# loehnea/bensolve

Hardware: AMD Instinct MI355X
Metric: scalar LPs/sec (Benson phase 2, batched P2(v) solves incl. cut application), synthetic VLP q=5 n=500 m=1000 (higher is better)
Workload: dtype f64

## Files before the change

### bensolve_amd/csrc/poly_engine.hip

```cpp
#include "common.h"
#include <vector>
#include <chrono>
#include <algorithm>
#include <cmath>
#include <thread>
#include <atomic>
#include <cstddef>

namespace bslv {

constexpr int MAXD = 16;
constexpr double POLY_EPS = 1e-9;
constexpr int PB = 256;
constexpr unsigned char F_USED = 1, F_IDEAL = 2, F_SLTN = 4;
constexpr int CRING = 1024;
constexpr int CSTRIDE = 8;
constexpr int LCAP = 16;
constexpr int LONGN = 64;
constexpr int ZMAX = 8;

struct Hp { double h[MAXD + 1]; };
struct Tri { int a, b, c; };

struct PolyView {
// ... 1387 lines not shown
                    if (it * WAVE >= nn) break;
                    const unsigned long long bm = __ballot(k[it]);
                    if (k[it]) {
                        P.pool[on + base + __popcll(bm & ((1ull << lane) - 1ull))] = g[it];
                        if (!row) P.keep[oo + it * WAVE + lane] = 0;
                        if (lb) atomicOr(&lb[g[it] >> 5], 1u << (g[it] & 31));
                    }
                    base += __popcll(bm);
                }
            } else
            for (int j0 = 0; j0 < nn; j0 += WAVE) {
                const int j = j0 + lane;
                const int g = j < nn ? P.pool[oo + j] : 0;
                const bool k = j < nn && (row ? row[g] == Z.stamp : P.keep[oo + j] != 0);
                const unsigned long long bm = __ballot(k);
                if (k) {
                    P.pool[on + base + __popcll(bm & ((1ull << lane) - 1ull))] = g;
                    if (!row) P.keep[oo + j] = 0;
                    if (lb) atomicOr(&lb[g >> 5], 1u << (g & 31));
                }
                base += __popcll(bm);
            }
            if (lane == 0) {
                P.pool[on + base] = facet; P.inc_off[vv] = on; P.inc_len[vv] = base + 1; if (lb) atomicOr(&lb[facet >> 5], 1u << (facet & 31));
                if (rm > 0) P.capx[vv] = ((unsigned long long)on << 32) | (unsigned)rm;
            }
        }
    }
    if (!valid) return;
    if (c == -1) { P.flag[i] &= ~F_USED; return; }
    if (c != 0) return;
    members[ex.a] = i;
    if (longz) return;
    int m = 0;
    if (n <= LCAP) {
        int lst[LCAP];
        unsigned keptmask = 0;
        const unsigned char *K = P.keep + off_old;
        load_list(P.pool + off_old, n, lst);
#pragma unroll
        for (int j = 0; j < LCAP; j++) { unsigned k = (j < n) ? K[j] : 0; keptmask |= (k & 1u) << j; }
#pragma unroll
        for (int j = 0; j < LCAP; j++) if ((keptmask >> j) & 1u) { P.pool[off_new + m++] = lst[j]; P.keep[off_old + j] = 0; }
    } else
        for (int j = 0; j < n; j++)
            if (P.keep[off_old + j]) { P.pool[off_new + m++] = P.pool[off_old + j]; P.keep[off_old + j] = 0; }
    P.pool[off_new + m++] = facet;
    P.inc_off[i] = off_new;
    P.inc_len[i] = m;
    relist_bitmap(P, i, off_new, m);
}

constexpr int K2T = 1024, K2_MAXNM = 512, K2_MAXLONG = 64;
constexpr int K2_HASH_LOG = 13, K2_HASH = 1 << K2_HASH_LOG;
__device__ __forceinline__ void pair_decode32(int p, int nm, int &i, int &j)
{
    const float b2 = 2.0f * nm - 1.0f;
    int ii = (int)((b2 - sqrtf(b2 * b2 - 8.0f * (float)p)) * 0.5f);
    ii = ii < 0 ? 0 : (ii > nm - 2 ? nm - 2 : ii);
    while (ii * (2 * nm - ii - 1) / 2 > p) ii--;
    while ((ii + 1) * (2 * nm - ii - 2) / 2 <= p) ii++;
    i = ii;
    j = ii + 1 + (p - ii * (2 * nm - ii - 1) / 2);
}
template <class F>
__device__ __forceinline__ void k2_for_entries(const int *pool, int nm, const unsigned *s_off, const int *s_len, const unsigned char *s_islong,
                                               const int *s_long, int nlong, F f)
{
    for (int m = threadIdx.x / LPM; m < nm; m += K2T / LPM) {
        if (s_islong[m]) continue;
        const int *L = pool + s_off[m];
        const int n = s_len[m];
        for (int j = threadIdx.x % LPM; j < n; j += LPM) f(m, L[j]);
    }
    for (int k = 0; k < nlong; k++) {
        const int m = s_long[k];
        const int *L = pool + s_off[m];
        const int n = s_len[m];
        for (int j = threadIdx.x; j < n; j += K2T) f(m, L[j]);
    }
}
template <int NWC>
__device__ __forceinline__ void k2_pairs(int nm, int d, int W, int NW, const unsigned long long *bits, const unsigned long long *rows, unsigned *adj_bits,
                                         int (*queue)[128], const unsigned long long *later = nullptr)
{
    const int lane = threadIdx.x & 63, wave = threadIdx.x >> 6;
    auto sweep = [&](int p) {
        int i, j;
        pair_decode32(p, nm, i, j);
        unsigned long long acc[NWC];
#pragma unroll
        for (int k = 0; k < NWC; k++) acc[k] = ~0ull;
        for (int w = 0; w < W; w++) {
            unsigned long long M = bits[w * nm + i] & bits[w * nm + j];
            while (M) {
                const int f = (w << 6) + __ffsll((long long)M) - 1;
                M &= M - 1;
#pragma unroll
                for (int k = 0; k < NWC; k++) acc[k] &= (NWC == 1 || k < NW) ? rows[f * NW + k] : 0ull;
            }
        }
        int cnt = 0;
#pragma unroll
        for (int k = 0; k < NWC; k++) cnt += __popcll(acc[k]);
        if (cnt == 2) atomicOr(&adj_bits[p >> 5], 1u << (p & 31));
    };
    int qn = 0;
    int *q = queue[wave];
    for (int i = wave; i < nm - 1; i += K2T / WAVE) {
        const int rowbase = i * (2 * nm - i - 1) / 2 - (i + 1);
        for (int j0 = i + 1; j0 < nm; j0 += WAVE) {
            const int j = j0 + lane;
            bool cand = false;
            if (j < nm) {
                int nmut = 0;
                unsigned long long lat = 0ull;
                for (int w = 0; w < W; w++) { const unsigned long long x = bits[w * nm + i] & bits[w * nm + j]; nmut += __popcll(x); if (later) lat |= x & later[w]; }
                if (d == 1) atomicOr(&adj_bits[(rowbase + j) >> 5], 1u << ((rowbase + j) & 31));
                else cand = nmut >= d - 1 && lat == 0ull;
            }
            const unsigned long long bm = __ballot(cand);
            if (bm == 0ull) continue;
            if (cand) q[qn + __popcll(bm & ((1ull << lane) - 1ull))] = rowbase + j;
            qn += __popcll(bm);
            __builtin_amdgcn_fence(__ATOMIC_SEQ_CST, "wavefront");
            if (qn >= WAVE) {
                qn -= WAVE;
                sweep(q[qn + lane]);
                __builtin_amdgcn_fence(__ATOMIC_SEQ_CST, "wavefront");
            }
        }
    }
    if (lane < qn) sweep(q[lane]);
}
struct RState;
struct K2V2 {
    const RState *st; const int *cutof; int *mem_g; unsigned *adj_g; int *cnt_g; int *nm_g; int adjw_cap; long long *pair_tests;
    int *fc2, *fl2, *fc_ticket; int fc_slices, fc_stride;
};
__device__ __forceinline__ int k2v2_round(const RState *st);
__device__ __forceinline__ int k2v2_rank_base(const RState *st);
__device__ __forceinline__ bool k2v2_member(const PolyView &P, int v, int co, int vs, int want)
{
    if (co >= -1) return co == vs;
    const int k = -1 - co;
    const int *tail = P.pool + P.inc_off[v] + P.inc_len[v] - k;
    bool mine = false;
    for (int t = 0; t < k; t++) mine |= tail[t] == want;
    return mine;
}
__device__ __forceinline__ void k2v2_sizes(const RState *st, int &S, int &go, int &nzero, int &nv0, int &ncross);
__device__ void k2v2_check_members(const K2V2 &V, int vs, const int *s_mem, int nm, const int *members, int nzero);
template <bool V2>
__device__ void k2_fused_body(PolyView P, int *members, int nzero, int nv0, int ncross, int *fcount, int *flocal,
                              int lds_words, int2 *E, int ebase, int *ne_dev, Tri *totals, Mail *mail, int seq, unsigned long long *dbg,
                              const CutDev *cd, int *abort_flag, int *EP, const Hp &hn, int *counters_n, int *zlist_n, const K2V2 &V)
{
    extern __shared__ unsigned long long k2_dyn[];
    if (V2) {
        int S, go;
        k2v2_sizes(V.st, S, go, nzero, nv0, ncross);
        if (blockIdx.x == 0 && threadIdx.x == 0 && V.fc_ticket) V.fc_ticket[(k2v2_round(V.st) + 1) & 1] = 0;
        if (!go || (int)blockIdx.x >= S) return;
        cd = nullptr; ne_dev = nullptr;
    }
    if (!V2 && blockIdx.x > 0) {
        classify_body(P, hn, cd->nv_new, counters_n, zlist_n, (blockIdx.x - 1) * K2T + threadIdx.x);
        return;
    }
    if (cd) {
        nzero = cd->nzero; ncross = cd->ncross; ebase = cd->ebase;
        const int nm_ = nzero + ncross;
        if (!cd->go || nm_ < 2 || nm_ > K2_MAXNM) {
            if (threadIdx.x == 0) {
                const bool big = cd->go && nm_ > K2_MAXNM;
                Tri r{0, big ? 1 : 2, 0};
                if (big) *abort_flag = 1;
                totals[0] = r;
                if (ne_dev) *ne_dev = ebase;
                mail->t = r;
                mail->seq = seq;
            }
            return;
        }
    }
    unsigned long long t_prev = dbg ? wall_clock64() : 0ull;
#define K2_PHASE(k) do { if (dbg && threadIdx.x == 0) { unsigned long long t_now = wall_clock64(); if (V2) atomicAdd(&dbg[k], t_now - t_prev); else dbg[k] += t_now - t_prev; t_prev = t_now; } } while (0)
    __shared__ Tri lds[16];
    __shared__ unsigned s_off[K2_MAXNM];
    __shared__ int s_len[K2_MAXNM], s_mem[K2_MAXNM], s_long[K2_MAXLONG];
    __shared__ unsigned char s_islong[K2_MAXNM];
    __shared__ int s_nlong, s_nloc, s_carry;
    __shared__ int s_queue[K2T / WAVE][128];
    const int tid = threadIdx.x, d = P.d;
    int nm = nzero + ncross;
    const int vs = (int)blockIdx.x;
    const int myrank = V2 ? k2v2_rank_base(V.st) + vs : 0x7FFFFFFF;
    auto v2_result = [&](int cnt, int n) { if (tid == 0) { V.cnt_g[vs] = cnt; V.nm_g[vs] = n; } };
    if (V2) {
        __shared__ int s_base;
        if (tid == 0) s_base = 0;
        __syncthreads();
        const int ncand = nzero + ncross;
        constexpr int CPT = 8;
        for (int c0 = 0; c0 < ncand; c0 += K2T * CPT) {
            const int cb = c0 + tid * CPT;
            int vv[CPT], co[CPT], cnt = 0;
#pragma unroll
            for (int u = 0; u < CPT; u++) { const int c = cb + u; vv[u] = c < ncand ? (c < nzero ? members[c] : nv0 + (c - nzero)) : -1; }
#pragma unroll
            for (int u = 0; u < CPT; u++) co[u] = vv[u] >= 0 ? V.cutof[vv[u]] : 0;
#pragma unroll
            for (int u = 0; u < CPT; u++) { if (vv[u] >= 0 && !k2v2_member(P, vv[u], co[u], vs, myrank)) vv[u] = -1; cnt += vv[u] >= 0; }
            Tri t{cnt, 0, 0};
            Tri tot;
            const Tri ex = block_exscan(t, &tot, lds);
            int pos = s_base + ex.a;
#pragma unroll
            for (int u = 0; u < CPT; u++) if (vv[u] >= 0) { if (pos < K2_MAXNM) s_mem[pos] = vv[u]; pos++; }
            __syncthreads();
            if (tid == 0) s_base += tot.a;
            __syncthreads();
        }
        nm = s_base;
        K2_PHASE(10);
        if (nm > K2_MAXNM) { v2_result(-1, nm); return; }
#ifdef BSLV_R2_CHECK_MEMBERS
        k2v2_check_members(V, vs, s_mem, nm, members, nzero);
#endif
        if (tid == 0 && nm >= 2) atomicAdd((unsigned long long *)V.pair_tests, (unsigned long long)((long long)nm * (nm - 1) / 2));
        if (nm < 2) { v2_result(0, nm); return; }
    }
    const long long npairs = (long long)nm * (nm - 1) / 2;
    const int nadjw = (int)((npairs + 31) / 32);
    unsigned *adj_bits = (unsigned *)k2_dyn;
    unsigned long long *bits = k2_dyn + (nadjw + 1) / 2;
    const long long bits_cap = (long long)lds_words - (nadjw + 1) / 2;
    if (bits_cap < 0) {
        if (V2) { v2_result(-2, nm); return; }
        if (threadIdx.x == 0) { Tri r{0, 1, 0}; totals[0] = r; if (ne_dev) *ne_dev = ebase; if (abort_flag) *abort_flag = 1; mail->t = r; mail->seq = seq; }
        return;
    }
    for (int m = tid; m < nm; m += K2T) {
        int v;
        if (V2) v = s_mem[m];
        else if (m < nzero) v = members[m]; else { v = nv0 + (m - nzero); members[m] = v; }
        s_mem[m] = v; s_off[m] = P.inc_off[v]; s_len[m] = P.inc_len[v]; s_islong[m] = 0;
    }
    for (int w = tid; w < nadjw; w += K2T) adj_bits[w] = 0u;
    if (tid == 0) { s_nlong = 0; s_nloc = 0; s_carry = 0; }
    __syncthreads();
    for (int m = tid; m < nm; m += K2T)
        if (s_len[m] > LONGN) { int k = atomicAdd(&s_nlong, 1); if (k < K2_MAXLONG) { s_long[k] = m; s_islong[m] = 1; } }
    __syncthreads();
    const int nlong = s_nlong < K2_MAXLONG ? s_nlong : K2_MAXLONG;
    K2_PHASE(0);
    __shared__ int s_total;
    if (tid == 0) s_total = 0;
    __syncthreads();
    {
        int part = 0;
        for (int m = tid; m < nm; m += K2T) part += s_len[m];
#pragma unroll
        for (int o = 32; o > 0; o >>= 1) part += __shfl_xor(part, o, WAVE);
        if ((tid & 63) == 0 && part) atomicAdd(&s_total, part);
    }
    __syncthreads();
    const bool use_hash = 2 * s_total <= K2_HASH && (long long)K2_HASH <= bits_cap;
    if (V2 && !use_hash) {
        __shared__ int s_slice;
        if (tid == 0) s_slice = V.fc_slices > 0 ? atomicAdd(&V.fc_ticket[k2v2_round(V.st) & 1], 1) : V.fc_slices;
        __syncthreads();
        if (s_slice >= V.fc_slices) { v2_result(-3, nm); return; }
        fcount = V.fc2 + (size_t)s_slice * V.fc_stride;
        flocal = V.fl2 + (size_t)s_slice * V.fc_stride;
    }
    int *hkey = (int *)bits, *hval = hkey + K2_HASH;
    if (use_hash) bits += K2_HASH;
    const long long bcap = use_hash ? bits_cap - K2_HASH : bits_cap;
    auto hslot = [&](int g) {
        unsigned sl = ((unsigned)g * 2654435761u) >> (32 - K2_HASH_LOG);
        for (;;) {
            const int k = atomicCAS(&hkey[sl], -1, g);
            if (k == -1 || k == g) return (int)sl;
            sl = (sl + 1) & (K2_HASH - 1);
        }
    };
    if (use_hash) {
        for (int w = tid; w < K2_HASH; w += K2T) { hkey[w] = -1; hval[w] = 0; }
        __syncthreads();
        k2_for_entries(P.pool, nm, s_off, s_len, s_islong, s_long, nlong, [&](int, int g) { atomicAdd(&hval[hslot(g)], 1); });
        __syncthreads();
        for (int w = tid; w < K2_HASH; w += K2T) hval[w] = hval[w] >= 2 ? (0x40000000 | atomicAdd(&s_nloc, 1)) : 0;
        __syncthreads();
    } else {
        k2_for_entries(P.pool, nm, s_off, s_len, s_islong, s_long, nlong, [&](int, int g) {
            if (atomicAdd(&fcount[g], 1) == 1) __hip_atomic_store(&flocal[g], atomicAdd(&s_nloc, 1), __ATOMIC_RELAXED, __HIP_MEMORY_SCOPE_AGENT);
        });
        __threadfence_block();
        __syncthreads();
    }
    K2_PHASE(1);
    K2_PHASE(2);
    const int W = (s_nloc + 63) >> 6, NW = (nm + 63) >> 6;
    unsigned long long *rows = bits + W * nm;
    unsigned long long *later = rows + W * 64 * NW;
    if (V2 && (long long)W * nm + (long long)W * 64 * NW + W > bcap) {
        if (!use_hash) k2_for_entries(P.pool, nm, s_off, s_len, s_islong, s_long, nlong, [&](int, int g) { fcount[g] = 0; });
        v2_result(-4, nm);
        return;
    }
    if ((long long)W * nm + (long long)W * 64 * NW > bcap) {
        if (!use_hash) k2_for_entries(P.pool, nm, s_off, s_len, s_islong, s_long, nlong, [&](int, int g) { fcount[g] = 0; });
        if (tid == 0) { Tri r{0, 1, 0}; totals[0] = r; if (ne_dev) *ne_dev = ebase; if (abort_flag) *abort_flag = 1; mail->t = r; mail->seq = seq; }
        return;
    }
    for (int w = tid; w < W * nm + W * 64 * NW + (V2 ? W : 0); w += K2T) bits[w] = 0ull;
    __syncthreads();
    if (use_hash)
        k2_for_entries(P.pool, nm, s_off, s_len, s_islong, s_long, nlong, [&](int m, int g) {
            const int v = hval[hslot(g)];
            if (!(v & 0x40000000)) return;
            const int id = v & 0x3FFFFFFF;
            atomicOr(&bits[(id >> 6) * nm + m], 1ull << (id & 63));
            atomicOr(&rows[id * NW + (m >> 6)], 1ull << (m & 63));
            if (V2 && g > myrank) atomicOr(&later[id >> 6], 1ull << (id & 63));
        });
    else
        k2_for_entries(P.pool, nm, s_off, s_len, s_islong, s_long, nlong, [&](int m, int g) {
            if (__hip_atomic_load(&fcount[g], __ATOMIC_RELAXED, __HIP_MEMORY_SCOPE_AGENT) < 2) return;
            const int id = __hip_atomic_load(&flocal[g], __ATOMIC_RELAXED, __HIP_MEMORY_SCOPE_AGENT);
            atomicOr(&bits[(id >> 6) * nm + m], 1ull << (id & 63));
            atomicOr(&rows[id * NW + (m >> 6)], 1ull << (m & 63));
            if (V2 && g > myrank) atomicOr(&later[id >> 6], 1ull << (id & 63));
        });
    __syncthreads();
    if (!use_hash) k2_for_entries(P.pool, nm, s_off, s_len, s_islong, s_long, nlong, [&](int, int g) { fcount[g] = 0; });
    K2_PHASE(3);
    const unsigned long long *lat = V2 ? later : nullptr;
    if (NW <= 1) k2_pairs<1>(nm, d, W, NW, bits, rows, adj_bits, s_queue, lat);
    else if (NW <= 2) k2_pairs<2>(nm, d, W, NW, bits, rows, adj_bits, s_queue, lat);
    else if (NW <= 4) k2_pairs<4>(nm, d, W, NW, bits, rows, adj_bits, s_queue, lat);
    else k2_pairs<K2_MAXNM / 64>(nm, d, W, NW, bits, rows, adj_bits, s_queue, lat);
    __syncthreads();
    K2_PHASE(4);
    K2_PHASE(5);
    if (V2) {
        unsigned *ag = V.adj_g + (size_t)vs * V.adjw_cap;
        int *mg = V.mem_g + (size_t)vs * K2_MAXNM;
        int part = 0;
        for (int w = tid; w < nadjw; w += K2T) { const unsigned x = adj_bits[w]; ag[w] = x; part += __popc(x); }
        for (int m = tid; m < nm; m += K2T) mg[m] = s_mem[m];
        const Tri tt = block_sum(Tri{part, 0, 0}, lds);
        v2_result(tt.a, nm);
        K2_PHASE(6);
        if (dbg && tid == 0) { atomicAdd(&dbg[7], 1ull); atomicAdd(&dbg[8], (unsigned long long)W); atomicAdd(&dbg[9], (unsigned long long)s_nloc); atomicAdd(&dbg[11], (unsigned long long)nm); atomicMax(&dbg[12], (unsigned long long)nm); }
        return;
    }
    int last_tot = 0;
    for (int w0 = 0; w0 < nadjw; w0 += K2T) {
        const int ww = w0 + tid;
        unsigned word = ww < nadjw ? adj_bits[ww] : 0u;
        Tri t{(int)__popc(word), 0, 0};
        Tri tot;
        Tri ex = block_exscan(t, &tot, lds);
        int at = ebase + s_carry + ex.a;
        while (word) {
            const int bbit = __ffs((int)word) - 1;
            word &= word - 1;
            int i, j;
            pair_decode32(ww * 32 + bbit, nm, i, j);
            E[at] = int2{s_mem[i], s_mem[j]};
            if (EP) EP[at] = -1;
            at++;
        }
        if (w0 + K2T < nadjw) {
            __syncthreads();
            if (tid == 0) s_carry += tot.a;
            __syncthreads();
        } else last_tot = tot.a;
    }
    K2_PHASE(6);
    if (tid == 0) {
        if (dbg) { dbg[7] += 1; dbg[8] += (unsigned long long)W; dbg[9] += (unsigned long long)s_nloc; }
        Tri r{s_carry + last_tot, 0, 0};
        totals[0] = r;
        if (ne_dev) *ne_dev = ebase + r.a;
        mail->t = r;
        mail->seq = seq;
    }
}


template <bool V2>
__global__ __launch_bounds__(K2T) void k2_fused_t(PolyView P, int *members, int nzero, int nv0, int ncross, int *fcount, int *flocal,
                                                  int lds_words, int2 *E, int ebase, int *ne_dev, Tri *totals, Mail *mail, int seq, unsigned long long *dbg,
                                                  const CutDev *cd, int *abort_flag, int *EP, Hp hn, int *counters_n, int *zlist_n, K2V2 V)
{
    k2_fused_body<V2>(P, members, nzero, nv0, ncross, fcount, flocal, lds_words, E, ebase, ne_dev, totals, mail, seq, dbg, cd, abort_flag, EP, hn, counters_n, zlist_n, V);
}

__global__ void k_forward_mail(const Mail *src, Mail *dst)
{
    const Tri t = src->t;
    mail_publish(dst, nullptr, t, src->seq);
}

struct HotElems : CompactOp {
    PolyView P; const int *tc; int *hv;
    __device__ __forceinline__ Tri pick(int i) const { return Tri{(P.flag[i] & F_USED) && tc[i] > 0, 0, 0}; }
    __device__ __forceinline__ void seen_emit(int i, const Tri &t) const { if (!t.a) P.cls[i] = 1; }
    __device__ __forceinline__ void put(int i, int pos, const Tri &) const { hv[pos] = i; }
};
__global__ __launch_bounds__(PB) void k_lbits_build(PolyView P, int nhv, int maxslots, int *nslots)
{
    const int idx = blockIdx.x * (PB / WAVE) + (threadIdx.x >> 6), lane = threadIdx.x & 63;
    if (idx >= nhv) return;
    const int v = P.hv[idx], n = P.inc_len[v];
    if (n <= LONGN) return;
    int sl = 0;
    if (lane == 0) sl = atomicAdd(nslots, 1);
    sl = __shfl(sl, 0, WAVE);
    if (sl >= maxslots) return;
    unsigned *row = P.lbits + (size_t)sl * P.lstride;
    const int *L = P.pool + P.inc_off[v];
    for (int j = lane; j < n; j += WAVE) { const int g = L[j]; atomicOr(&row[g >> 5], 1u << (g & 31)); }
    if (lane == 0) P.lslot[v] = sl;
}
__global__ void k_lbits_reset(PolyView P, int nhv)
{
    const int idx = blockIdx.x * blockDim.x + threadIdx.x;
    if (idx < nhv) P.lslot[P.hv[idx]] = -1;
}
struct HotEdge : Tri { int2 ed; };
struct HotEdges : CompactOp {
    const int2 *E; const int *tc; int2 *EH; int *EP; unsigned char *alive;
    __device__ __forceinline__ HotEdge pick(int e) const { const int2 ed = E[e]; return HotEdge{{tc[ed.x] > 0 || tc[ed.y] > 0, 0, 0}, ed}; }
    __device__ __forceinline__ void seen_emit(int e, const HotEdge &t) const { alive[e] = t.a ? 0 : 1; }
    __device__ __forceinline__ void put(int e, int pos, const HotEdge &t) const { EH[pos] = t.ed; EP[pos] = e; }
// ... 141 lines not shown
        const int cnj = D.flen[cj];
        const int *pool = P.pool + P.inc_off[cv];
        const int npool = P.inc_len[cv];
        bool found = false;
        for (int base = 0; base < npool; base += WAVE) {
            int k = base + lane;
            bool hit = false;
            if (k < npool) {
                int w = pool[k];
                if (w != fi && w != cj && D.flive[w] && D.flen[w] >= cn)
                    hit = isect3_count(A, ni, cL, cnj, D.fpool + D.foff[w], D.flen[w]) == cn;
            }
            if (__ballot(hit)) { found = true; break; }
        }
        if (lane == src) adj = !found;
    }
    Tri t{adj ? 1 : 0, 0, 0};
    pflag[(size_t)blockIdx.x * PB + threadIdx.x] = adj ? 1 : 0;
    Tri tot;
    (void)block_exscan(t, &tot, lds);
    if (threadIdx.x == 0) bsum[blockIdx.x] = tot;
}


__global__ __launch_bounds__(PB) void k_live_ranks(PolyView P, int nv, unsigned char *live)
{
    const int i = blockIdx.x * (PB / WAVE) + (threadIdx.x >> 6), lane = threadIdx.x & 63;
    if (i >= nv || !(P.flag[i] & F_USED)) return;
    const int *L = P.pool + P.inc_off[i];
    const int n = P.inc_len[i];
    for (int j = lane; j < n; j += WAVE) live[L[j]] = 1;
}
__global__ void k_bench_fill(PolyView P, int nv, unsigned long long seed)
{
    int i = blockIdx.x * blockDim.x + threadIdx.x;
    if (i >= nv) return;
    for (int k = 0; k < P.d; k++) {
        unsigned long long z = seed + 0x9E3779B97F4A7C15ull * ((unsigned long long)i * P.d + k + 1);
        z = (z ^ (z >> 30)) * 0xBF58476D1CE4E5B9ull;
        z = (z ^ (z >> 27)) * 0x94D049BB133111EBull;
        z ^= z >> 31;
        P.X[(size_t)k * P.cap + i] = (double)(z >> 11) * (1.0 / 9007199254740992.0) * 2.0 - 1.0;
    }
    P.flag[i] = F_USED;
    P.inc_len[i] = 0;
    P.inc_off[i] = 0;
}
#include "poly_rounds_kernels.inc"
#include "poly_rounds2_kernels.inc"
__device__ void k2v2_check_members(const K2V2 &V, int vs, const int *s_mem, int nm, const int *members, int nzero)
{
    RState *st = const_cast<RState *>(V.st);
    for (int m = threadIdx.x; m < nm; m += blockDim.x)
        for (int m2 = m + 1; m2 < nm; m2++)
            if (s_mem[m] == s_mem[m2] && atomicCAS(&st->err, 0, 4) == 0) {
                int c1 = -1, c2 = -1;
                for (int c = 0; c < nzero; c++) if (members[c] == s_mem[m]) { if (c1 < 0) c1 = c; else c2 = c; }
                st->err_info[0] = vs; st->err_info[1] = m; st->err_info[2] = m2; st->err_info[3] = s_mem[m]; st->err_info[4] = c1; st->err_info[5] = c2; st->err_info[6] = nzero;
            }
}
__device__ __forceinline__ int k2v2_round(const RState *st) { return st->round; }
__device__ __forceinline__ int k2v2_rank_base(const RState *st) { return st->rank_base; }
__device__ __forceinline__ void k2v2_sizes(const RState *st, int &S, int &go, int &nzero, int &nv0, int &ncross)
{
    S = st->S; go = st->go && !r2_halted(st); nzero = st->nzero; nv0 = st->nv; ncross = st->ncross;
}


}

using namespace bslv;

struct RoundsBuf;
struct Rounds2Buf;
struct bslv_poly {
    RoundsBuf *rounds = nullptr;
    Rounds2Buf *rounds2 = nullptr;
    bool rounds2_enabled = true;
    bool r2_spec = true;
    long r2_spec_void = 0;
    bool r2_mis = true;
    bool r2_ride = true;
    int r2_ride_gmax = 240;
    int r2_ride_threads = 256;
    int chunk_cuts = 1024;
    int r2_defer = 0;
    bool r2_deferred = false;
    long r2_deferred_cuts = 0, r2_doomed = 0;
    bool r2_defer_mark = !(getenv("BSLV_DEFER_MARK") && atoi(getenv("BSLV_DEFER_MARK")) == 0);
    bool snap = false;
    unsigned long long *snapped_d = nullptr;
    int r2_min_cuts = 0;
    long r2_rounds = 0, r2_cuts = 0, r2_fallback_prunes = 0, r2_declined = 0, r2_chunks = 0, shuffle_seq = 0, r2_late_left = 0, r2_torn_reads = 0;
    long r2_fb_reason[5] = {0, 0, 0, 0, 0}, r2_fb_nm[20] = {0};
    int batch_mode = 1;
    long rounds_run = 0, conf_pairs = 0, conf_cuts = 0;
    int dense_streak = 0, dense_skip = 0;
    int d = 0, v2h = 0;
    std::vector<double> c;
    hipStream_t stream = nullptr;
    PolyView P{};
    int nv = 0;
    unsigned poolcap = 0, poolused = 0;
    int2 *E[2] = {nullptr, nullptr};
    int ecap = 0, ne = 0, ecur = 0;
    unsigned char *eflag = nullptr;
    int *ecount = nullptr; int ecountcap = 0;
    int *EP[2] = {nullptr, nullptr};
    bool hot = false, hot_enabled = true;
    struct EdgeSet { int2 *E[2] = {nullptr, nullptr}; int *EP[2] = {nullptr, nullptr}; unsigned char *eflag = nullptr; int ecap = 0, ne = 0, ecur = 0; } full, hotbuf;
    unsigned char *alive = nullptr; int alivecap = 0;
    int *hv_d = nullptr; int hvcap = 0;
    int *lslot_d = nullptr; int lslotcap = 0;
    unsigned *lbits_d = nullptr; size_t lbitscap = 0; int *lnslots_d = nullptr;
    long hot_chunks = 0, hot_elems = 0, hot_edges = 0;
    long n_spec = 0, n_declined = 0, n_k2_fallback = 0, n_single = 0;
    double tm_hot_begin = 0, tm_seq = 0, tm_hot_end = 0, tm_add_cuts = 0; long tm_seq_cuts = 0;
    double tm_realloc = 0; long n_realloc = 0;
    double tm_prep = 0, tm_classify_wait = 0, tm_newdual = 0;
    double tm_launch[4] = {0, 0, 0, 0};
    int *members = nullptr;
    Tri *bsum = nullptr; int bsumcap = 0;
    Tri *bsum2 = nullptr; size_t bsum2cap = 0;
    int *fm_cnt = nullptr, *fm_list = nullptr; size_t fmcap = 0, fmlistcap = 0; int fm_min = 4096; long n_fm = 0; bool member_lists = true;
    int largest_facet = 0;
    bool k2_noflags = getenv("BSLV_K2_NOFLAGS") != nullptr; long n_noflag_prunes = 0;
    long long window_blocks = 0x7FFFFFF0ll, win_max_blocks = 0; long n_win_prunes = 0, n_windows = 0;
    int shard_min = 32768; long n_sharded = 0; int2 *shard_e = nullptr; size_t shardcap = 0;
    int *nzlist = nullptr; size_t nzcap = 0;
    Tri *totals = nullptr;
    int *counters = nullptr;
    Tri *totals_h = nullptr; int *counters_h = nullptr;
    Mail *mail_h = nullptr, *mail_d = nullptr;
    Mail mail_v[4];
    long mail_torn_reads = 0;
    Mail *k2mail_d = nullptr;
    int *fstamp = nullptr, *flocal = nullptr, *nlocal = nullptr; int fcap = 0;
    unsigned long long *bits = nullptr; size_t bitscap = 0;
    int mailseq = 0;
    long cutseq = 0;
    size_t k2_lds = 0;
    int *ne_dev = nullptr;
    bool pend_k2 = false;
    int pend_seq = 0, pend_slot = 2, pend_ebase = 0, pend_nm = 0, pend_stamp = 0, pend_nzero = 0, pend_nv0 = 0, pend_ncross = 0; long long pend_len_ub = 0;
    int k2flip = 0;
    bool speculate = true;
    int cross_ub = CROSS_UB;
    CutDev *cutdev = nullptr;
    int *abort_d = nullptr;
    int *fcount = nullptr;
    int *zlist = nullptr, *zrows = nullptr;
    int pre_f = -1, pre_slot = 0, pre_nv = 0, pre_seq = 0;
    unsigned long long *k2dbg = nullptr;
    FILE *cutlog = nullptr;
    PairBlk *blks = nullptr; int blkcap = 0;
    unsigned char *pflag = nullptr; size_t pflagcap = 0;
    std::vector<double> Y, hp;
    std::vector<unsigned char> fapplied, fideal;
    std::vector<int> facet_of_rank;
    int nf = 0;
    bool initialised = false;
    std::vector<int> queue;
    std::vector<int> dual_edges;
    long pair_tests = 0, new_vertices = 0, cuts_applied = 0;
    double *hps_d = nullptr; int hpscap = 0; std::vector<double> hps_stage;
    unsigned long long *clsw = nullptr; size_t clswcap = 0;
// ... 772 lines not shown
    HIP_TRY(hipMemcpy(h->P.inc_off, off.data(), n * sizeof(unsigned), hipMemcpyHostToDevice));
    HIP_TRY(hipMemcpy(h->P.inc_len, len.data(), n * sizeof(int), hipMemcpyHostToDevice));
    HIP_TRY(hipMemcpy(h->P.pool, pool.data(), pool.size() * sizeof(int), hipMemcpyHostToDevice));
    h->poolused = (unsigned)pool.size();
    std::vector<int2> E;
    for (int k = 0; k <= d; k++) for (int j = k + 1; j <= d; j++) E.push_back(int2{k, j});
    HIP_TRY(hipMemcpy(h->E[h->ecur], E.data(), E.size() * sizeof(int2), hipMemcpyHostToDevice));
    h->ne = (int)E.size();
    h->nv = n;
    h->facet_of_rank.resize(h->nf);
    for (int f = 0; f < h->nf; f++) h->facet_of_rank[f] = f;
    return 0;
}

static double gs_step(const double *x, double *H, double *R, int k, int n)
{
    double nrm_in = 0, scl = 0;
    for (int l = 0; l < n; l++) nrm_in += x[l] * x[l];
    nrm_in = std::sqrt(nrm_in);
    double *hr = H + (size_t)k * n;
    for (int l = 0; l < n; l++) hr[l] = x[l];
    for (int j = 0; j < k; j++) {
        double s = 0;
        for (int l = 0; l < n; l++) s += H[(size_t)j * n + l] * hr[l];
        for (int l = 0; l < n; l++) hr[l] -= s * H[(size_t)j * n + l];
    }
    for (int l = 0; l < n; l++) scl += hr[l] * hr[l];
    scl = std::sqrt(scl);
    if (scl < 1.0e-6) return 0;
    for (int l = 0; l < n; l++) hr[l] /= scl;
    for (int j = 0; j <= k; j++) {
        double s = 0;
        for (int l = 0; l < n; l++) s += H[(size_t)j * n + l] * x[l];
        R[k * (k + 1) / 2 + j] = s;
    }
    return scl / nrm_in;
}

extern "C" {

int bslv_poly_create(bslv_poly **out, int dim, int v2h, const double *c)
{
    if (!out || dim < 2 || dim > MAXD || v2h < 0 || v2h > 2) { set_error("bslv_poly_create: bad argument (2 <= dim <= %d)", MAXD); return BSLV_E_ARG; }
    if (bslv_device_count() < 1) { set_error("no HIP device available"); return BSLV_E_NODEVICE; }
    bslv_poly *h = new bslv_poly();
    h->d = dim; h->v2h = v2h;
    h->c.assign(dim, 0.0);
    if (c) h->c.assign(c, c + dim);
    h->P.d = dim;
    auto fail = [&](int code) { bslv_poly_destroy(h); return code; };
    if (hipStreamCreate(&h->stream) != hipSuccess) { set_error("hipStreamCreate failed"); return fail(BSLV_E_NODEVICE); }
    if (malloc0(&h->totals, 4 * sizeof(Tri)) != hipSuccess || malloc0(&h->counters, CRING * CSTRIDE * sizeof(int)) != hipSuccess || malloc0(&h->ne_dev, 4 * sizeof(int)) != hipSuccess || malloc0(&h->k2mail_d, 4 * sizeof(Mail)) != hipSuccess || hipMemset(h->k2mail_d, 0, 4 * sizeof(Mail)) != hipSuccess || malloc0(&h->cutdev, CRING * sizeof(CutDev)) != hipSuccess ||
        malloc0(&h->abort_d, 4 * sizeof(int)) != hipSuccess || hipMemset(h->abort_d, 0, 4 * sizeof(int)) != hipSuccess || malloc0(&h->zlist, CRING * ZMAX * sizeof(int)) != hipSuccess ||
        hipHostMalloc(&h->totals_h, 4 * sizeof(Tri)) != hipSuccess || hipHostMalloc(&h->counters_h, 4 * sizeof(int)) != hipSuccess ||
        hipHostMalloc(&h->mail_h, 4 * sizeof(Mail), hipHostMallocMapped | hipHostMallocCoherent) != hipSuccess ||
        hipHostGetDevicePointer((void **)&h->mail_d, h->mail_h, 0) != hipSuccess ||
        hipMemset(h->counters, 0, CRING * CSTRIDE * sizeof(int)) != hipSuccess) {
        set_error("allocation of scan scratch failed");
        return fail(BSLV_E_NOMEM);
    }
    memset((void *)h->mail_h, 0, 4 * sizeof(Mail));
    memset((void *)h->mail_v, 0, sizeof h->mail_v);
    for (int k = 0; k < 4; k++) h->mail_h[k].chk2 = mail_sum2(Tri{0, 0, 0}, 0);
    h->k2_lds = 128 * 1024;
    if (hipFuncSetAttribute((const void *)k2_fused_t<false>, hipFuncAttributeMaxDynamicSharedMemorySize, (int)h->k2_lds) != hipSuccess ||
        hipFuncSetAttribute((const void *)k2_fused_t<true>, hipFuncAttributeMaxDynamicSharedMemorySize, (int)h->k2_lds) != hipSuccess) {
        (void)hipGetLastError();
        h->k2_lds = 48 * 1024;
    }
    if (const char *cl = getenv("BSLV_CUT_LOG")) h->cutlog = fopen(cl, "w");
    if (getenv("BSLV_NO_SPEC")) h->speculate = false;
    if (getenv("BSLV_NO_HOT")) h->hot_enabled = false;
    if (getenv("BSLV_NO_ROUNDS2")) h->rounds2_enabled = false;
    if (const char *e = getenv("BSLV_R2_MIS")) h->r2_mis = atoi(e) != 0;
    if (const char *e = getenv("BSLV_R2_SPEC")) h->r2_spec = atoi(e) != 0;
    {
        int dev = 0, cus = 0;
        if (hipGetDevice(&dev) == hipSuccess && hipDeviceGetAttribute(&cus, hipDeviceAttributeMultiprocessorCount, dev) == hipSuccess && cus > 0) h->r2_ride_gmax = std::max(cus / 2, cus - 16);
        else (void)hipGetLastError();
    }
    if (const char *e = getenv("BSLV_R2_RIDE")) h->r2_ride = atoi(e) != 0;
    if (const char *e = getenv("BSLV_R2_RIDE_G")) h->r2_ride_gmax = std::max(1, atoi(e));
    if (const char *e = getenv("BSLV_R2_RIDE_T")) bslv_poly_debug_set(h, 20, atol(e));
    if (const char *e = getenv("BSLV_CHUNK_CUTS")) h->chunk_cuts = std::min(4096, std::max(32, atoi(e)));
    if (const char *e = getenv("BSLV_R2_MIN_CUTS")) h->r2_min_cuts = std::max(-1, atoi(e));
    if (const char *e = getenv("BSLV_POLY_SNAP")) h->snap = atoi(e) != 0;
    if (const char *e = getenv("BSLV_CROSS_UB")) h->cross_ub = std::max(0, atoi(e));
    if (const char *e = getenv("BSLV_K2_LDS")) h->k2_lds = (size_t)std::max(64, atoi(e));
    if (const char *e = getenv("BSLV_K2_WINDOW")) { const long long v = atoll(e); if (v > 0) h->window_blocks = std::min(v, PAIR_WINDOW_DEFAULT); }
    if (getenv("BSLV_K2_DEBUG") && malloc0(&h->k2dbg, 16 * sizeof(unsigned long long)) == hipSuccess) (void)hipMemset(h->k2dbg, 0, 16 * sizeof(unsigned long long));
    h->rounds = new RoundsBuf();
    std::vector<double> z(dim, 0.0);
    z[dim - 1] = -1.0;
    new_dual(h, z.data(), 1);
    *out = h;
    return 0;
}

void bslv_poly_destroy(bslv_poly *h)
{
    if (!h) return;
    if (getenv("BSLV_R2_REPORT") && h->r2_fallback_prunes) {
        fprintf(stderr, "r2: %ld prunes of rounds went through the multi-kernel path: %ld members > %d, %ld pair bitmap, %ld hash table, %ld bit matrix | members by power of two:", h->r2_fallback_prunes,
                h->r2_fb_reason[1], K2_MAXNM, h->r2_fb_reason[2], h->r2_fb_reason[3], h->r2_fb_reason[4]);
        for (int k = 0; k < 20; k++) if (h->r2_fb_nm[k]) fprintf(stderr, " 2^%d: %ld", k, h->r2_fb_nm[k]);
        fprintf(stderr, "\n");
    }
    if (getenv("BSLV_TIMING"))
        fprintf(stderr, "poly timing: add_cuts %.1f ms | hot_begin %.1f, sequences %.1f (%ld cuts, %.1f us each), hot_end %.1f ms | %ld hot chunks, %.0f elements, %.0f edges on average\n", h->tm_add_cuts,
                h->tm_hot_begin, h->tm_seq, h->tm_seq_cuts, h->tm_seq_cuts ? h->tm_seq * 1e3 / h->tm_seq_cuts : 0.0, h->tm_hot_end, h->hot_chunks,
                h->hot_chunks ? (double)h->hot_elems / h->hot_chunks : 0.0, h->hot_chunks ? (double)h->hot_edges / h->hot_chunks : 0.0),
        fprintf(stderr, "poly timing, per batch of cuts: dual slots %.2f ms, chunk preparation %.2f ms, waiting for the batched classification %.2f ms (totals); %ld re-allocations of element / edge / pool arrays, %.2f ms\n", h->tm_newdual, h->tm_prep, h->tm_classify_wait, h->n_realloc, h->tm_realloc),
        fprintf(stderr, "poly host per cut (us): queue round A %.1f, k_emit2 %.1f, round B in all %.1f, mailbox wait %.1f\n", h->tm_launch[0] / std::max(1L, h->n_single), h->tm_launch[1] / std::max(1L, h->n_single),
                h->tm_launch[2] / std::max(1L, h->n_single), h->tm_launch[3] / std::max(1L, h->n_single));
    if (h->cutlog) fclose(h->cutlog);
    if (h->k2dbg) {
        unsigned long long t[16];
        if (hipMemcpy(t, h->k2dbg, sizeof(t), hipMemcpyDeviceToHost) == hipSuccess && t[7])
            fprintf(stderr, "k2_fused phases (us/launch over %llu launches; rounds: per prune workgroup): P0a %.2f P0 %.2f P1 %.2f P2 %.2f P3 %.2f P4 %.2f P5 %.2f P6 %.2f | W %.1f nloc %.0f | members mean %.0f max %llu\n", t[7],
                    t[10] * 0.01 / t[7], t[0] * 0.01 / t[7], t[1] * 0.01 / t[7], t[2] * 0.01 / t[7], t[3] * 0.01 / t[7], t[4] * 0.01 / t[7], t[5] * 0.01 / t[7], t[6] * 0.01 / t[7], (double)t[8] / t[7], (double)t[9] / t[7],
                    (double)t[11] / t[7], t[12]);
        (void)hipFree(h->k2dbg);
    }
    auto fr = [](void *p) { if (p) (void)hipFree(p); };
    fr(h->P.X); fr(h->P.flag); fr(h->P.cls); fr(h->P.inc_off); fr(h->P.inc_len); fr(h->P.capx); fr(h->P.pool); fr(h->P.keep);
    fr(h->E[0]); fr(h->E[1]); fr(h->eflag); fr(h->members); fr(h->bsum); fr(h->bsum2); fr(h->fm_cnt); fr(h->fm_list); fr(h->nzlist); fr(h->totals); fr(h->counters); fr(h->ne_dev); fr(h->k2mail_d); fr(h->zlist); fr(h->zrows); fr(h->fcount); fr(h->cutdev); fr(h->abort_d);
    for (int k = 0; k < 2; k++) { fr(h->hotbuf.E[k]); fr(h->hotbuf.EP[k]); }
    fr(h->snapped_d);
    fr(h->hotbuf.eflag); fr(h->alive); fr(h->hv_d); fr(h->ecount); fr(h->lslot_d); fr(h->lbits_d); fr(h->lnslots_d);
    fr(h->shard_e); fr(h->blks); fr(h->pflag); fr(h->fstamp); fr(h->flocal); fr(h->nlocal); fr(h->bits); fr(h->hps_d); fr(h->clsw); fr(h->live_d); fr(h->anyminus); fr(h->idx_d); fr(h->val_d); fr(h->fl_d); fr(h->par_d); fr(h->r2f_d); fr(h->fhist_d); fr(h->chosen_d); fr(h->cmp_d);
    if (h->rounds) { rounds_free(*h->rounds); delete h->rounds; }
    if (h->rounds2) { rounds2_free(*h->rounds2); delete h->rounds2; }
    if (h->totals_h) (void)hipHostFree(h->totals_h);
    if (h->counters_h) (void)hipHostFree(h->counters_h);
    if (h->mail_h) (void)hipHostFree((void *)h->mail_h);
    if (h->stream) (void)hipStreamDestroy(h->stream);
    delete h;
}

int bslv_poly_dual0_apex(bslv_poly *h)
{
    if (!h) return BSLV_E_ARG;
    h->fideal[0] = 0;
    h->Y[h->d - 1] = 0.0;
    v2h_map(h, h->Y.data(), 0, h->hp.data());
    return 0;
}

int bslv_poly_add(bslv_poly *h, const double *val, int ideal, int *rc_out)
{
    if (!h || !val || !rc_out) { set_error("bslv_poly_add: bad argument"); return BSLV_E_ARG; }
    int f = new_dual(h, val, ideal);
    if (!h->initialised) { h->queue.push_back(f); *rc_out = 0; return 0; }
    int rc = do_cut(h, f, rc_out);
    return rc ? rc : settle_k2(h);
}

int bslv_poly_init(bslv_poly *h, int *rc_out)
{
    if (!h || !rc_out) return BSLV_E_ARG;
    if (h->initialised) { set_error("bslv_poly_init: already initialised"); return BSLV_E_STATE; }
    const int d = h->d;
    int qn = (int)h->queue.size();
    if (qn < d) { *rc_out = 1; return 0; }
    std::vector<double> hpq((size_t)qn * (d + 1));
    for (int k = 0; k < qn; k++) memcpy(&hpq[(size_t)k * (d + 1)], &h->hp[(size_t)h->queue[k] * (d + 1)], (d + 1) * sizeof(double));
    std::vector<double> H((size_t)d * d, 0.0), R((size_t)d * (d + 1) / 2, 0.0), alph(d, 0.0);
    std::vector<int> perm(d + 1, 0);
    int g = 0;
    while (g < d) {
        double best = 0; int bi = -1;
        for (int k = 0; k < qn; k++) {
            double s = gs_step(&hpq[(size_t)k * (d + 1)], H.data(), R.data(), g, d);
            if (best < s) { best = s; bi = k; }
        }
        if (best < 1.0e-10) { *rc_out = 1; return 0; }
        gs_step(&hpq[(size_t)bi * (d + 1)], H.data(), R.data(), g, d);
        alph[g] = hpq[(size_t)bi * (d + 1) + d];
        perm[++g] = h->queue[bi];
        qn--;
        memcpy(&hpq[(size_t)bi * (d + 1)], &hpq[(size_t)qn * (d + 1)], (d + 1) * sizeof(double));
        h->queue[bi] = h->queue[qn];
    }
    auto RM = [&](int k, int j) -> double & { return R[k * (k + 1) / 2 + j]; };
    std::vector<double> X((size_t)(d + 1) * d, 0.0), t(d, 0.0);
    for (int k = 0; k < d; k++) {
        double s = alph[k];
        for (int j = 0; j < k; j++) s -= RM(k, j) * t[j];
        t[k] = s / RM(k, k);
    }
    for (int j = 0; j < d; j++) { double s = 0; for (int l = 0; l < d; l++) s += H[(size_t)l * d + j] * t[l]; X[j] = s; }
    for (int k = 0; k < d; k++) {
        std::fill(t.begin(), t.end(), 0.0);
        t[k] = 1.0 / RM(k, k);
        for (int i = k + 1; i < d; i++) {
            double s = 0;
            for (int j = k; j < i; j++) s += RM(i, j) * t[j];
            t[i] = -s / RM(i, i);
        }
        for (int j = 0; j < d; j++) { double s = 0; for (int l = 0; l < d; l++) s += H[(size_t)l * d + j] * t[l]; X[(size_t)(k + 1) * d + j] = s; }
    }
// ... 262 lines not shown
}
int bslv_poly_children_of(bslv_poly *h, int nfacets, const int *facets, int max_out, int *idx, double *val, int *ideal, int *parent, int *n_out)
{
    if (!h || nfacets < 0 || (nfacets > 0 && !facets) || max_out < 0 || !n_out || (max_out > 0 && !idx)) { set_error("bslv_poly_children_of: bad argument"); return BSLV_E_ARG; }
    *n_out = 0;
    if (!h->initialised || h->nv == 0 || nfacets == 0 || max_out == 0) return 0;
    hipStream_t s = h->stream;
    int rc;
    const int nv = h->nv, nf = h->nf;
    int f0 = nf;
    for (int k = 0; k < nfacets; k++) { if (facets[k] < 0 || facets[k] >= nf) { set_error("bslv_poly_children_of: facet %d out of range", facets[k]); return BSLV_E_ARG; } f0 = std::min(f0, facets[k]); }
    std::vector<unsigned char> chosen((size_t)(nf - f0), 0);
    for (int k = 0; k < nfacets; k++) chosen[facets[k] - f0] = 1;
    if ((rc = sync_r2f(h))) return rc;
    if ((size_t)(nf - f0) > h->chosencap) { const size_t nc = std::max((size_t)(nf - f0) + 4096, h->chosencap * 2); if ((rc = grow(&h->chosen_d, 0, nc, s))) return rc; h->chosencap = nc; }
    HIP_TRY(hipMemcpyAsync(h->chosen_d, chosen.data(), chosen.size(), hipMemcpyHostToDevice, s));
    UnprocChosen op{{}, h->P, h->r2f_d, h->chosen_d, f0, {}};
    Tri t;
    if ((rc = compact_count(h, op, nv, &t))) return rc;
    const int n = std::min(t.a, max_out);
    if (n == 0) return 0;
    if ((rc = ensure_out(h, n))) return rc;
    op.out = UnprocOut{t.a - n, n, 0, h->idx_d, h->val_d, h->fl_d, h->par_d};
    if ((rc = compact_emit(h, op, nv))) return rc;
    std::vector<unsigned char> fl(n);
    if ((rc = fetch_out(h, n, idx, val, parent, fl.data(), ideal))) return rc;
    *n_out = n;
    return 0;
}

int bslv_poly_next(bslv_poly *h, double *val, int *ideal, int *idx, int *rc_out)
{
    if (!h || !val || !ideal || !idx || !rc_out) return BSLV_E_ARG;
    int cnt = 0;
    int rc = bslv_poly_unprocessed(h, 1, idx, val, ideal, &cnt);
    if (rc) return rc;
    *rc_out = cnt > 0 ? 0 : 1;
    return 0;
}

int bslv_poly_mark(bslv_poly *h, int n, const int *idx)
{
    if (!h || n < 0 || (n > 0 && !idx)) return BSLV_E_ARG;
    if (n == 0) return 0;
    for (int k = 0; k < n; k++) if (idx[k] < 0 || idx[k] >= h->nv) { set_error("bslv_poly_mark: slot %d out of range", idx[k]); return BSLV_E_ARG; }
    int rc;
    if ((rc = ensure_out(h, n))) return rc;
    HIP_TRY(hipMemcpyAsync(h->idx_d, idx, n * sizeof(int), hipMemcpyHostToDevice, h->stream));
    hipLaunchKernelGGL(k_mark, dim3((n + 255) / 256), dim3(256), 0, h->stream, h->P, h->idx_d, n, F_SLTN);
    HIP_TRY(hipGetLastError());
    HIP_TRY(hipStreamSynchronize(h->stream));
    return 0;
}

int bslv_poly_set_batch_mode(bslv_poly *h, int mode)
{
    if (!h || mode < 0 || mode > 1) return BSLV_E_ARG;
    h->batch_mode = mode;
    return 0;
}
long bslv_poly_rounds_run(const bslv_poly *h) { return h ? h->rounds_run : 0; }
int bslv_poly_set_defer(bslv_poly *h, int min_cuts)
{
    if (!h || min_cuts < 0) return BSLV_E_ARG;
    h->r2_defer = min_cuts;
    return 0;
}
int bslv_poly_debug_set(bslv_poly *h, int key, long value)
{
    if (!h) return BSLV_E_ARG;
    switch (key) {
    case 0: h->k2_lds = (size_t)std::max(64L, value); return 0;
    case 1: h->speculate = value != 0; return 0;
    case 2: h->hot_enabled = value != 0; return 0;
    case 3: h->cross_ub = (int)std::max(0L, value); return 0;
    case 4: h->fm_min = (int)std::max(2L, value); return 0;
    case 6: h->rounds2_enabled = value != 0; return 0;
    case 7: h->chunk_cuts = (int)std::min(4096L, std::max(32L, value)); return 0;
    case 10: h->shard_min = (int)std::max(2L, value); return 0;
    case 12: h->r2_spec = value != 0; return 0;
    case 18: h->r2_ride = value != 0; return 0;
    case 19: h->r2_ride_gmax = (int)std::max(1L, std::min(4096L, value)); return 0;
    case 20: { int t = 64; while (t < K2T && t < value) t <<= 1; h->r2_ride_threads = t; return 0; }
    case 16: h->k2_noflags = value != 0; return 0;
    case 11: h->r2_mis = value != 0; return 0;
    case 14: h->r2_defer = (int)std::max(0L, value); return 0;
    case 8: h->r2_min_cuts = (int)std::max(-1L, value); return 0;
    case 21: h->cmp_keep_cap = value != 0; return 0;
    case 5: h->member_lists = value != 0; return 0;
    default: return BSLV_E_ARG;
    }
}
long bslv_poly_sharded_prunes(const bslv_poly *h) { return h ? h->n_sharded : 0; }
int bslv_poly_set_snap(bslv_poly *h, int on)
{
    if (!h) return BSLV_E_ARG;
    if (h->hot) { set_error("bslv_poly_set_snap: a chunk of cuts is open"); return BSLV_E_ARG; }
    int rc = settle_k2(h);
    if (rc) return rc;
    h->pre_f = -1;
    h->snap = on != 0;
    return 0;
}
int bslv_poly_snapped(bslv_poly *h, long *moved)
{
    if (!h || !moved) return BSLV_E_ARG;
    unsigned long long v = 0;
    if (h->snapped_d) { HIP_TRY(hipStreamSynchronize(h->stream)); HIP_TRY(hipMemcpy(&v, h->snapped_d, sizeof(v), hipMemcpyDeviceToHost)); }
    *moved = (long)v;
    return 0;
}
int bslv_poly_largest_facet(const bslv_poly *h) { return h ? h->largest_facet : 0; }
long bslv_poly_noflag_prunes(const bslv_poly *h) { return h ? h->n_noflag_prunes : 0; }
int bslv_poly_set_prune_window(bslv_poly *h, long blocks)
{
    if (!h || blocks < 0) return BSLV_E_ARG;
    h->window_blocks = blocks == 0 ? PAIR_WINDOW_DEFAULT : std::min<long long>(blocks, PAIR_WINDOW_DEFAULT);
    return 0;
}
long bslv_poly_get_prune_window(const bslv_poly *h) { return h ? (long)h->window_blocks : 0; }
int bslv_poly_prune_window_stats(const bslv_poly *h, long out[3])
{
    if (!h || !out) return BSLV_E_ARG;
    out[0] = h->n_win_prunes; out[1] = h->n_windows; out[2] = (long)h->win_max_blocks;
    return 0;
}
int bslv_selftest_pair_blocks(int nm, long window_blocks, int samples, long out[4])
{
    if (nm < 2 || window_blocks < 0 || samples < 1 || !out) return BSLV_E_ARG;
    const long long wb = window_blocks == 0 ? PAIR_WINDOW_DEFAULT : std::min<long long>(window_blocks, PAIR_WINDOW_DEFAULT);
    const long long total = pair_G(nm - 1);
    std::vector<PairWin> wins;
    pair_windows(nm, wb, wins);
    long long at = 0, wmax = 0; int g = 0;
    for (const PairWin &w : wins) {
        const long long one = pair_S(nm, (long long)(w.g0 + 1) * PTI) - w.vb0;
        if (w.g0 != g || w.g1 <= w.g0 || w.vb0 != at || w.nb < 1 || w.nb > std::max(wb, one) || w.nb - 1 >= (1ll << 31)) {
            set_error("pair windows of %d members: window [%d, %d) at block %lld with %lld blocks breaks the table (expected group %d at block %lld, at most %lld blocks)",
                      nm, w.g0, w.g1, w.vb0, w.nb, g, at, std::max(wb, one));
            return BSLV_E_STATE;
        }
        g = w.g1; at += w.nb; wmax = std::max(wmax, w.nb);
    }
    if (g != (nm - 1 + PTI - 1) / PTI || at != total) { set_error("pair windows of %d members cover %lld of %lld blocks", nm, at, total); return BSLV_E_STATE; }
    std::vector<long long> vb0s(wins.size());
    for (size_t k = 0; k < wins.size(); k++) vb0s[k] = wins[k].vb0;
    long long *vb0_d = nullptr; unsigned long long *bad_d = nullptr, bad = 0;
    auto cleanup = [&]() { if (vb0_d) (void)hipFree(vb0_d); if (bad_d) (void)hipFree(bad_d); };
    if (hipMalloc((void **)&vb0_d, vb0s.size() * sizeof(long long)) != hipSuccess || hipMalloc((void **)&bad_d, sizeof(unsigned long long)) != hipSuccess) {
        cleanup(); set_error("bslv_selftest_pair_blocks: allocation failed"); return BSLV_E_NOMEM;
    }
    hipError_t e = hipMemcpy(vb0_d, vb0s.data(), vb0s.size() * sizeof(long long), hipMemcpyHostToDevice);
    if (e == hipSuccess) e = hipMemset(bad_d, 0, sizeof(unsigned long long));
    if (e == hipSuccess) {
        hipLaunchKernelGGL(k_selftest_pair_blocks, dim3((unsigned)((samples + PB - 1) / PB)), dim3(PB), 0, 0, nm, (const long long *)vb0_d, (int)wins.size(), samples, bad_d);
        e = hipGetLastError();
    }
    if (e == hipSuccess) e = hipMemcpy(&bad, bad_d, sizeof bad, hipMemcpyDeviceToHost);
    cleanup();
    if (e != hipSuccess) { set_error("bslv_selftest_pair_blocks: %s", hipGetErrorString(e)); return BSLV_E_NODEVICE; }
    out[0] = (long)wins.size(); out[1] = (long)total; out[2] = (long)bad; out[3] = (long)(wmax - 1);
    return 0;
}
long bslv_poly_rounds2_late_left(const bslv_poly *h) { return h ? h->r2_late_left : 0; }
long bslv_poly_rounds2_torn_reads(const bslv_poly *h) { return h ? h->r2_torn_reads + h->mail_torn_reads : 0; }

int bslv_selftest_mailbox(int which, int rounds, long *torn_out)
{
    if (rounds < 1 || which < 0 || which > 1) return BSLV_E_ARG;
    long torn = 0, bad = 0;
    std::atomic<int> ack{0};
    if (which == 0) {
        Mail *box = new Mail();
        memset((void *)box, 0, sizeof *box);
        box->chk2 = mail_sum2(Tri{0, 0, 0}, 0);
        volatile Mail *m = box;
        std::thread writer([&] {
            for (int q = 1; q <= rounds; q++) {
                while (ack.load(std::memory_order_acquire) != q - 1) { }
                const int c4[4] = {q, 2 * q, 3 * q, 4 * q};
                const Tri t{5 * q, 6 * q, 7 * q}, k2{8 * q, 9 * q, 10 * q};
                m->seq = q;
                __sync_synchronize();
                for (int k = 0; k < 4; k++) { m->cnt[k] = c4[k]; for (volatile int d = 0; d < 50; d++) { } }
                const_cast<Mail *>(box)->t = t; const_cast<Mail *>(box)->k2t = k2; m->k2seq = 11 * q;
                for (volatile int d = 0; d < 200; d++) { }
                m->chk2 = mail_sum2(k2, 11 * q);
                m->chk = mail_sum(c4, t, q);
            }
        });
        for (int q = 1; q <= rounds; q++) {
            Mail got;
            while (!mail_try_read(m, q, &got, &torn)) { }
            if (got.cnt[0] != q || got.cnt[3] != 4 * q || got.t.a != 5 * q || got.t.c != 7 * q || got.k2t.b != 9 * q || got.k2seq != 11 * q) bad++;
            ack.store(q, std::memory_order_release);
        }
        writer.join();
        delete box;
    } else {
        RState *box = new RState();
        memset((void *)box, 0, sizeof *box);
        volatile RState *m = box;
        std::thread writer([&] {
            for (int q = 1; q <= rounds; q++) {
                while (ack.load(std::memory_order_acquire) != q - 1) { }
                RState st;
                memset((void *)&st, 0, sizeof st);
                st.round = q; st.S = 3 * q; st.nalive = 5 * q; st.napplied = 7 * q; st.ne_next = 11 * q; st.err_d[11] = 13.0 * q;
                st.chk = rstate_sum(st, q);
                m->seq = q;
                __sync_synchronize();
                const unsigned *src = reinterpret_cast<const unsigned *>(&st);
                volatile unsigned *dst = reinterpret_cast<volatile unsigned *>(box);
                const size_t seq_word = offsetof(RState, seq) / 4, chk_word = offsetof(RState, chk) / 4;
                for (size_t w = 0; w < sizeof(RState) / 4; w++) { if (w == seq_word || w == chk_word) continue; dst[w] = src[w]; for (volatile int d = 0; d < 10; d++) { } }
                dst[chk_word] = st.chk;
            }
        });
        for (int q = 1; q <= rounds; q++) {
            RState got;
            while (!rstate_try_read(m, q, &got, &torn)) { }
            if (got.round != q || got.S != 3 * q || got.nalive != 5 * q || got.napplied != 7 * q || got.ne_next != 11 * q || got.err_d[11] != 13.0 * q) bad++;
            ack.store(q, std::memory_order_release);
        }
        writer.join();
        delete box;
    }
    if (torn_out) *torn_out = torn;
    return bad ? (int)(-1 - bad) : 0;
}
int bslv_poly_path_stats(const bslv_poly *h, long out[6])
{
    if (!h || !out) return BSLV_E_ARG;
    out[0] = h->hot_chunks; out[1] = h->n_spec; out[2] = h->n_declined; out[3] = h->n_k2_fallback; out[4] = h->n_single; out[5] = h->n_fm;
    return 0;
}
long bslv_poly_conflict_pairs(const bslv_poly *h) { return h ? h->conf_pairs : 0; }
int bslv_poly_rounds2_stats(const bslv_poly *h, long out[5])
{
    if (!h || !out) return BSLV_E_ARG;
    out[0] = h->r2_rounds; out[1] = h->r2_cuts; out[2] = h->r2_chunks; out[3] = h->r2_fallback_prunes; out[4] = h->r2_declined;
    return 0;
}
int bslv_poly_bench_fill(bslv_poly *h, int nv, unsigned long long seed)
{
    if (!h || nv < 1) return BSLV_E_ARG;
    int rc;
    if ((rc = ensure_vcap(h, nv))) return rc;
    hipLaunchKernelGGL(k_bench_fill, dim3((nv + 255) / 256), dim3(256), 0, h->stream, h->P, nv, seed);
    HIP_TRY(hipGetLastError());
    HIP_TRY(hipStreamSynchronize(h->stream));
    h->nv = nv; h->ne = 0; h->initialised = true;
    if (h->facet_of_rank.empty()) h->facet_of_rank.push_back(0);
    return 0;
}

int bslv_poly_dim(const bslv_poly *h) { return h ? h->d : 0; }
int bslv_poly_nprimal(const bslv_poly *h) { return h ? h->nv : 0; }
int bslv_poly_ndual(const bslv_poly *h) { return h ? h->nf : 0; }
long bslv_poly_nedges(const bslv_poly *h) { return h ? h->ne : 0; }
long bslv_poly_pair_tests(const bslv_poly *h) { return h ? h->pair_tests : 0; }
long bslv_poly_new_vertices(const bslv_poly *h) { return h ? h->new_vertices : 0; }

int bslv_poly_get_primal_range(bslv_poly *h, int first, int count, double *coords)
{
    if (!h || first < 0 || count < 0 || first + count > h->nv || (count && !coords)) { set_error("bslv_poly_get_primal_range: bad argument"); return BSLV_E_ARG; }
    if (count == 0) return 0;
    const int d = h->d;
    std::vector<double> col(count);
    for (int k = 0; k < d; k++) {
        HIP_TRY(hipMemcpy(col.data(), h->P.X + (size_t)k * h->P.cap + first, (size_t)count * sizeof(double), hipMemcpyDeviceToHost));
        for (int i = 0; i < count; i++) coords[(size_t)i * d + k] = col[i];
    }
    return 0;
}
int bslv_poly_get_primal(bslv_poly *h, unsigned char *used, unsigned char *ideal, unsigned char *sltn, double *coords)
{
    if (!h) return BSLV_E_ARG;
    const int nv = h->nv, d = h->d;
    if (nv == 0) return 0;
    std::vector<unsigned char> fl(nv);
    HIP_TRY(hipMemcpy(fl.data(), h->P.flag, nv, hipMemcpyDeviceToHost));
    for (int i = 0; i < nv; i++) {
        if (used) used[i] = (fl[i] & F_USED) ? 1 : 0;
        if (ideal) ideal[i] = (fl[i] & F_IDEAL) ? 1 : 0;
        if (sltn) sltn[i] = (fl[i] & F_SLTN) ? 1 : 0;
    }
    if (coords) {
        std::vector<double> col(nv);
        for (int k = 0; k < d; k++) {
            HIP_TRY(hipMemcpy(col.data(), h->P.X + (size_t)k * h->P.cap, (size_t)nv * sizeof(double), hipMemcpyDeviceToHost));
            for (int i = 0; i < nv; i++) coords[(size_t)i * d + k] = col[i];
        }
    }
    return 0;
}

static int fetch_inc(bslv_poly *h, std::vector<unsigned char> &fl, std::vector<unsigned> &off, std::vector<int> &len, std::vector<int> &pool)
{
    const int nv = h->nv;
    fl.resize(nv); off.resize(nv); len.resize(nv); pool.resize(h->poolused);
    if (nv == 0) return 0;
    HIP_TRY(hipMemcpy(fl.data(), h->P.flag, nv, hipMemcpyDeviceToHost));
    HIP_TRY(hipMemcpy(off.data(), h->P.inc_off, nv * sizeof(unsigned), hipMemcpyDeviceToHost));
    HIP_TRY(hipMemcpy(len.data(), h->P.inc_len, nv * sizeof(int), hipMemcpyDeviceToHost));
    if (h->poolused) HIP_TRY(hipMemcpy(pool.data(), h->P.pool, (size_t)h->poolused * sizeof(int), hipMemcpyDeviceToHost));
    return 0;
}

long bslv_poly_ninc(bslv_poly *h)
{
    if (!h || h->nv == 0) return 0;
    std::vector<unsigned char> fl(h->nv);
    std::vector<int> len(h->nv);
    if (hipMemcpy(fl.data(), h->P.flag, h->nv, hipMemcpyDeviceToHost) != hipSuccess) return -1;
    if (hipMemcpy(len.data(), h->P.inc_len, h->nv * sizeof(int), hipMemcpyDeviceToHost) != hipSuccess) return -1;
    long n = 0;
    for (int i = 0; i < h->nv; i++) if (fl[i] & F_USED) n += len[i];
    return n;
}

int bslv_poly_get_inc(bslv_poly *h, int *pairs)
{
    if (!h || !pairs) return BSLV_E_ARG;
    std::vector<unsigned char> fl; std::vector<unsigned> off; std::vector<int> len, pool;
// ... 133 lines not shown
```

### bensolve_amd/csrc/poly_rounds2_host.inc

```
#include <string>
#include <deque>

struct Rounds2Buf {
    RState *st_d = nullptr;
    RState *mail_h = nullptr, *mail_d = nullptr;
    unsigned *alive = nullptr, *alive_prev = nullptr, *anym = nullptr, *bad = nullptr;
    int *selmap = nullptr, *sel = nullptr, *order = nullptr, *rcflag = nullptr;
    int bcap = 0;
    int *own = nullptr; int vcap = 0;
    unsigned long long *hw = nullptr; size_t hwcap = 0;
    int *cnt_g = nullptr, *nm_g = nullptr, *mem_g = nullptr; unsigned *adj_g = nullptr; int scap = 0;
    int *gout = nullptr, *gout_h = nullptr;
    int seq = 0;
    unsigned chunk_seed = 0;
    unsigned *M = nullptr, *selw = nullptr, *wm = nullptr; int *mcnt = nullptr; int wmcap = 0;
    int *fc2 = nullptr, *fl2 = nullptr, *fc_ticket = nullptr; int fc_slices = 0, fc_stride = 0;
    size_t ride_lds = 128 * 1024;
};
constexpr int R2_ADJW = (K2_MAXNM * (K2_MAXNM - 1) / 2 + 31) / 32;
constexpr int R2_MAILS = 4;

static void rounds2_free(Rounds2Buf &V)
{
    auto fr = [](void *p) { if (p) (void)hipFree(p); };
    fr(V.st_d); fr(V.alive); fr(V.alive_prev); fr(V.anym); fr(V.bad); fr(V.selmap); fr(V.sel); fr(V.order); fr(V.rcflag); fr(V.own);
    fr(V.cnt_g); fr(V.nm_g); fr(V.mem_g); fr(V.adj_g); fr(V.gout); fr(V.hw); fr(V.M); fr(V.selw); fr(V.wm); fr(V.mcnt); fr(V.fc2); fr(V.fl2); fr(V.fc_ticket);
    if (V.mail_h) (void)hipHostFree(V.mail_h);
    if (V.gout_h) (void)hipHostFree(V.gout_h);
    V = Rounds2Buf();
}
static hipError_t r2_prune_classify_grant(int d, int lds);
static int rounds2_ensure(bslv_poly *h, Rounds2Buf &V, int Bc)
{
    hipStream_t s = h->stream;
    int rc;
    if (!V.st_d) {
        HIP_TRY(malloc0(&V.st_d, sizeof(RState)));
        HIP_TRY(hipHostMalloc(&V.mail_h, R2_MAILS * sizeof(RState), hipHostMallocMapped | hipHostMallocCoherent));
        HIP_TRY(hipHostGetDevicePointer((void **)&V.mail_d, V.mail_h, 0));
        memset(V.mail_h, 0, R2_MAILS * sizeof(RState));
        HIP_TRY(malloc0(&V.gout, 4 * sizeof(int)));
        HIP_TRY(hipHostMalloc(&V.gout_h, 4 * sizeof(int)));
        HIP_TRY(malloc0(&V.M, (size_t)R2_MAXC * (R2_MAXC / 32) * sizeof(unsigned)));
        HIP_TRY(malloc0(&V.selw, 64 * sizeof(unsigned)));
        HIP_TRY(malloc0(&V.mcnt, (size_t)R2_MAXC * sizeof(int)));
        if (hipFuncSetAttribute((const void *)k_r2_select3, hipFuncAttributeMaxDynamicSharedMemorySize, (int)((R2_MAXC / 32) * R2_MLD * sizeof(unsigned))) != hipSuccess ||
            hipFuncSetAttribute((const void *)k_r2_minit, hipFuncAttributeMaxDynamicSharedMemorySize, (int)(((size_t)R2_MAXC * (R2_MAXC / 32 + 1) + R2_MAXC + 64) * sizeof(unsigned))) != hipSuccess) {
            (void)hipGetLastError();
            h->r2_mis = false;
        }
        if (r2_prune_classify_grant(h->d, 128 * 1024) != hipSuccess) { (void)hipGetLastError(); V.ride_lds = 48 * 1024; }
    }
    if (h->P.cap > V.wmcap) { if ((rc = grow(&V.wm, (size_t)V.wmcap, (size_t)h->P.cap, s, true))) return rc; V.wmcap = h->P.cap; }
    if (Bc > V.bcap) {
        const int nc = std::max(Bc, 1024), nw = (nc + 31) / 32 + 2;
        if ((rc = grow(&V.alive, 0, (size_t)nw, s))) return rc;
        if ((rc = grow(&V.alive_prev, 0, (size_t)nw, s))) return rc;
        if ((rc = grow(&V.anym, 0, (size_t)nw, s))) return rc;
        if ((rc = grow(&V.bad, 0, (size_t)nw, s))) return rc;
        if ((rc = grow(&V.selmap, 0, (size_t)nc, s))) return rc;
        if ((rc = grow(&V.sel, 0, (size_t)nc, s))) return rc;
        if ((rc = grow(&V.order, 0, (size_t)nc, s))) return rc;
        if ((rc = grow(&V.rcflag, 0, (size_t)nc, s))) return rc;
        if ((rc = grow(&V.cnt_g, 0, (size_t)nc, s))) return rc;
        if ((rc = grow(&V.nm_g, 0, (size_t)nc, s))) return rc;
        if ((rc = grow(&V.mem_g, 0, (size_t)nc * K2_MAXNM, s))) return rc;
        if ((rc = grow(&V.adj_g, 0, (size_t)nc * R2_ADJW, s))) return rc;
        V.bcap = nc; V.scap = nc;
    }
    if (h->P.cap > V.vcap) { if ((rc = grow(&V.own, 0, (size_t)h->P.cap, s))) return rc; V.vcap = h->P.cap; }
    return 0;
}
template <class... A>
static void launch_r2_emit(int d, dim3 grid, hipStream_t s, A... a)
{
    switch (d) {
#define CASE(D) case D: hipLaunchKernelGGL(k_r2_emit<D>, grid, dim3(PB), 0, s, a...); break;
        CASE(2) CASE(3) CASE(4) CASE(5) CASE(6) CASE(7) CASE(8) CASE(9) CASE(10)
#undef CASE
    default: hipLaunchKernelGGL(k_r2_emit<0>, grid, dim3(PB), 0, s, a...); break;
    }
}
template <class... A>
static void launch_r2_classify3(int d, dim3 grid, hipStream_t s, A... a)
{
    switch (d) {
#define CASE(D) case D: hipLaunchKernelGGL(k_r2_classify3<D>, grid, dim3(PB), 0, s, a...); break;
        CASE(2) CASE(3) CASE(4) CASE(5) CASE(6) CASE(7) CASE(8) CASE(9) CASE(10)
#undef CASE
    default: hipLaunchKernelGGL(k_r2_classify3<0>, grid, dim3(PB), 0, s, a...); break;
    }
}
template <class... A>
static void launch_r2_prune_classify(int d, dim3 grid, size_t lds, hipStream_t s, A... a)
{
    switch (d) {
#define CASE(D) case D: hipLaunchKernelGGL(k_r2_prune_classify<D>, grid, dim3(K2T), lds, s, a...); break;
        CASE(2) CASE(3) CASE(4) CASE(5) CASE(6) CASE(7) CASE(8) CASE(9) CASE(10)
#undef CASE
    default: hipLaunchKernelGGL(k_r2_prune_classify<0>, grid, dim3(K2T), lds, s, a...); break;
    }
}
static hipError_t r2_prune_classify_grant(int d, int lds)
{
    switch (d) {
#define CASE(D) case D: return hipFuncSetAttribute((const void *)k_r2_prune_classify<D>, hipFuncAttributeMaxDynamicSharedMemorySize, lds);
        CASE(2) CASE(3) CASE(4) CASE(5) CASE(6) CASE(7) CASE(8) CASE(9) CASE(10)
#undef CASE
    default: return hipFuncSetAttribute((const void *)k_r2_prune_classify<0>, hipFuncAttributeMaxDynamicSharedMemorySize, lds);
    }
}
static inline bool rstate_try_read(const volatile RState *m, int seq, RState *out, long *torn)
{
    if (m->seq != seq) return false;
    __sync_synchronize();
    RState c;
    memcpy((void *)&c, (const void *)m, sizeof c);
    if (c.seq == seq) {
        const unsigned chk = c.chk;
        c.chk = 0; c.seq = 0;
        if (rstate_sum(c, seq) == chk) { c.chk = chk; c.seq = seq; *out = c; return true; }
    }
    if (torn) ++*torn;
    return false;
}
static int r2_wait(bslv_poly *h, Rounds2Buf &V, int seq, RState *out)
{
    volatile RState *m = V.mail_h + (seq % R2_MAILS);
    long torn = 0, drained = 0;
    for (long spin = 0; !rstate_try_read(m, seq, out, &torn); spin++) {
        if ((spin & 0xFFFF) == 0xFFFF) {
            hipError_t e = hipStreamQuery(h->stream);
            if (e == hipSuccess && ++drained > 1024) {
                set_error("poly engine: the round mailbox never reached a consistent state for seq %d (seq there: %d, %ld torn reads)", seq, (int)m->seq, torn);
                return BSLV_E_STATE;
            }
            if (e != hipSuccess && e != hipErrorNotReady) { set_error("poly engine: stream error %s", hipGetErrorString(e)); return BSLV_E_NODEVICE; }
        }
    }
    h->r2_torn_reads += torn;
    if (torn) { static const bool rep = getenv("BSLV_R2_REPORT") != nullptr; if (rep) fprintf(stderr, "r2: mailbox seq %d arrived before its state: %ld reads repeated\n", seq, torn); }
    return 0;
}

static int run_rounds2(bslv_poly *h, RoundsBuf &R, const std::vector<int> &todo, const std::vector<int> &fid_local, const std::vector<int> &rem, int *rc_out,
                       int Bc, int nw, std::vector<int> &left_out)
{
    left_out.clear();
    h->r2_deferred = false;
    if (!h->hot || h->pend_k2) { set_error("internal: run_rounds2 in the wrong state"); return BSLV_E_STATE; }
// ... 119 lines not shown
    int cur = h->ecur;
    int gv = 8192, ge = 16384;
    int max_dv = 0, max_de = 0;
    bool stop_enq = false;
    auto clear_halt = [&]() -> int { HIP_TRY(hipMemsetAsync(&V.st_d->halt, 0, 2 * sizeof(int), s)); return 0; };
    auto drain = [&]() -> int {
        while (!inflight.empty()) {
            RState x;
            if ((rc = r2_wait(h, V, inflight.front().first, &x))) return rc;
            inflight.pop_front();
            h->r2_spec_void++;
        }
        cur = h->ecur;
        return 0;
    };
    auto launch_round = [&](bool ahead, int *seq_out, int *sub_out) -> int {
        const int nv = h->nv + (ahead ? gv : 0), ne = h->ne + (ahead ? ge : 0);
        const int nbv = (vm_count(h->P, std::min(nv, h->P.cap)) + PB - 1) / PB, nbe = std::max(1, (std::min(ne, h->ecap) + PB - 1) / PB);
        Tri *ebsum = h->bsum, *vbsum = h->bsum + nbe + 1;
        const int cslot = next_counter_slot(h);
        if (cslot < 0) { set_error("hipMemsetAsync failed"); return BSLV_E_NODEVICE; }
        int *counters = h->counters + CSTRIDE * cslot;
        const ZMarks Z{h->zlist + ZMAX * cslot, h->zrows, h->fcap, (int)h->cutseq};
        const int2 *Eold = h->E[cur];
        int2 *Enew = h->E[1 - cur];
        if (mis) {
            {
                const int items = ne + vm_count(h->P, std::min(nv, h->P.cap));
                static const int wgmax = getenv("BSLV_R2_MINIT_WG") ? std::max(1, atoi(getenv("BSLV_R2_MINIT_WG"))) : 256;
                const int nwg = std::max(1, std::min(wgmax, (items + 1023) / 1024));
                static const int probe_at = getenv("BSLV_R2_MINIT_PROBE") ? atoi(getenv("BSLV_R2_MINIT_PROBE")) : -1;
                static int probe_n = 0;
                static unsigned long long *probe_d = nullptr;
                unsigned long long *probe = nullptr;
                if (probe_at >= 0) {
                    if (!probe_d) (void)hipMalloc(&probe_d, 256 * 16 * sizeof(unsigned long long));
                    const int pos = (int)rounds + (int)inflight.size();
                    if (probe_n++ >= probe_at && pos == (getenv("BSLV_R2_MINIT_PROBE_POS") ? atoi(getenv("BSLV_R2_MINIT_PROBE_POS")) : 0) && probe_n < 1000000) {
                        probe = probe_d; probe_n = 1000000;
                        (void)hipMemsetAsync(probe_d, 0, 256 * 16 * sizeof(unsigned long long), s);
                    }
                }
                hipLaunchKernelGGL(k_r2_minit, dim3(nwg), dim3(1024), ((size_t)Bc * (nw + 1) + Bc + nw) * sizeof(unsigned), s, h->P, (const unsigned long long *)V.hw, (const unsigned *)V.wm, nw, Bc,
                                   (const RState *)V.st_d, Eold, (const unsigned *)V.alive, V.M, V.mcnt, (const int *)R.tc, V.st_d, std::min(ne, h->ecap), vm_count(h->P, std::min(nv, h->P.cap)), probe);
                if (probe) {
                    std::vector<unsigned long long> pr(256 * 16);
                    (void)hipStreamSynchronize(s);
                    (void)hipMemcpy(pr.data(), probe_d, pr.size() * 8, hipMemcpyDeviceToHost);
                    unsigned long long t0 = ~0ull, t4 = 0;
                    for (int g = 0; g < nwg; g++) { t0 = std::min(t0, pr[g * 16]); t4 = std::max(t4, pr[g * 16 + 4]); }
                    fprintf(stderr, "minit probe: nwg %d items %d (ne %d) Bc %d nw %d round %d, whole %.1f us\n", nwg, items, ne, Bc, nw, (int)rounds + (int)inflight.size(), (t4 - t0) / 100.0);
                    const char *nm[4] = {"zero", "items", "queue", "or"};
                    for (int k = 0; k < 4; k++) {
                        double mn = 1e30, mx = 0, sm = 0;
                        for (int g = 0; g < nwg; g++) { const double d = (pr[g * 16 + k + 1] - pr[g * 16 + k]) / 100.0; mn = std::min(mn, d); mx = std::max(mx, d); sm += d; }
                        fprintf(stderr, "  %-6s min %.1f mean %.1f max %.1f us\n", nm[k], mn, sm / nwg, mx);
                    }
                    double st_mn = 1e30, st_mx = 0, qs = 0, qmx = 0, nz = 0;
                    for (int g = 0; g < nwg; g++) { const double d = (pr[g * 16] - t0) / 100.0; st_mn = std::min(st_mn, d); st_mx = std::max(st_mx, d); qs += pr[g * 16 + 6]; qmx = std::max(qmx, (double)pr[g * 16 + 6]); nz += pr[g * 16 + 7]; }
                    { double a = 0, b2 = 0, c = 0, d2 = 0; for (int g = 0; g < nwg; g++) { a += pr[g * 16 + 8]; b2 += pr[g * 16 + 9]; c += pr[g * 16 + 10]; d2 = std::max(d2, (double)pr[g * 16 + 11]); }
                      fprintf(stderr, "  per wave (mean over %d waves): resolve + first fetch %.1f us, giving %.1f us, waiting for the next item's words %.1f us; slowest wave %.1f us\n", nwg * 16, a / nwg / 16 / 100, b2 / nwg / 16 / 100, c / nwg / 16 / 100, d2 / 100); }
                    fprintf(stderr, "  start skew max %.1f us; queue items mean %.0f max %.0f; non-zero words per wg %.0f\n", st_mx, qs / nwg, qmx, nz / nwg);
                }
            }
            hipLaunchKernelGGL(k_r2_select3, dim3(1), dim3(1024), (size_t)nw * R2_MLD * sizeof(unsigned), s, Bc, nw, V.alive, V.alive_prev, V.M, V.mcnt,
                               V.selmap, V.sel, V.order, V.rcflag, V.st_d, V.selw, depth);
            hipLaunchKernelGGL(k_r2_assign3, dim3(nbv), dim3(PB), 0, s, h->P, (const unsigned long long *)V.hw, (const unsigned *)V.wm, nw, (const RState *)V.st_d, (const unsigned *)V.selw,
                               (const int *)V.selmap, R.cutof, counters, h->zlist + ZMAX * cslot);
        } else {
            hipLaunchKernelGGL(k_r2_prep, dim3(nbe + nbv), dim3(PB), (size_t)(3 * nw + 2) * sizeof(unsigned), s, h->P, (const unsigned long long *)V.hw, nw,
                               (const RState *)V.st_d, Eold, nbe, (const unsigned *)V.alive, V.anym, V.bad, V.own, (const int *)R.tc, V.st_d);
            hipLaunchKernelGGL(k_r2_select, dim3(1), dim3(1024), 0, s, Bc, V.alive, V.alive_prev, V.anym, V.bad, V.selmap, V.sel, V.order, V.rcflag, V.st_d, depth);
            hipLaunchKernelGGL(k_r2_assign, dim3(nbv), dim3(PB), 0, s, h->P, (const unsigned long long *)V.hw, nw, (const RState *)V.st_d, (const int *)V.own,
                               (const int *)V.selmap, R.cutof, counters, h->zlist + ZMAX * cslot);
        }
        hipLaunchKernelGGL(k_flags2, dim3(nbe + nbv), dim3(PB), 0, s, h->P, Eold, ne, (const int *)&V.st_d->ne, nbe, nv, (const int *)counters, h->eflag, h->ecount, ebsum, vbsum, Z, (const int *)&V.st_d->nv,
                           (const int *)&V.st_d->halt, mis ? R2Own{(const int *)R.cutof, (const unsigned long long *)V.hw, (const unsigned *)V.wm, (const unsigned *)V.selw, (const int *)V.selmap, nw}
                                                           : R2Own{nullptr, nullptr, nullptr, nullptr, nullptr, 0});
        launch_r2_emit(d, dim3(nbe + nbv), s, h->P, (const double *)h->hps_d, (const int *)V.sel, R.cutof, Eold, nbe, (const unsigned char *)h->eflag, (const int *)h->ecount,
                       (const Tri *)ebsum, (const Tri *)vbsum, Enew, h->members, (const int *)counters, V.st_d, h->P.cap, h->ecap, h->poolcap,
                       (const int *)h->EP[cur], h->EP[1 - cur], Z, (const unsigned long long *)V.hw, (const unsigned *)V.wm, nw, (int *)nullptr,
                       (const unsigned *)V.selw, (const int *)V.selmap);
        const int S_ub = std::max(1, std::min(Bc - napplied - nredundant, V.scap));
        const K2V2 KV{V.st_d, R.cutof, V.mem_g, V.adj_g, V.cnt_g, V.nm_g, R2_ADJW, &V.st_d->pair_tests, V.fc2, V.fl2, V.fc_ticket, V.fc2 ? V.fc_slices : 0, V.fc_stride};
        const int seq = ++V.seq;
        const int want = std::max(2048, 2 * last_ncross);
        if (h->r2_ride && h->k2_lds <= V.ride_lds) {
            const int nthr = std::max(h->r2_ride_threads, std::min(nwp, K2T));
            const int vpb = std::max(1, nthr / nwp), G = std::max(1, std::min(h->r2_ride_gmax, (want + vpb - 1) / vpb));
            launch_r2_prune_classify(d, dim3(S_ub + G), h->k2_lds, s, h->P, h->members, h->fcount, h->flocal, (int)(h->k2_lds / 8), Enew, h->totals + 2, h->k2mail_d, h->k2dbg, h->abort_d,
                                     Hp{}, KV, (const double *)h->hps_d, Bc, nw, nwp, (const unsigned *)V.alive, V.hw, V.wm, G, nthr, mis ? 1 : 0);
        } else {
            launch_r2_classify3(d, dim3(std::max(1, std::min(4096, (want + PB / nwp - 1) / (PB / nwp)))), s, h->P, (const double *)h->hps_d, Bc, nw, nwp, (const RState *)V.st_d,
                                (const unsigned *)V.alive, V.hw, V.wm, (int *)nullptr, mis ? 1 : 0);
            hipLaunchKernelGGL(k2_fused_t<true>, dim3(S_ub), dim3(K2T), h->k2_lds, s, h->P, h->members, 0, 0, 0, h->fcount, h->flocal, (int)(h->k2_lds / 8), Enew, 0,
                               (int *)nullptr, h->totals + 2, h->k2mail_d, 0, h->k2dbg, (const CutDev *)nullptr, h->abort_d, (int *)nullptr, Hp{}, (int *)nullptr,
                               (int *)nullptr, KV);
        }
        hipLaunchKernelGGL(k_r2_k2emit, dim3(S_ub), dim3(K2T), 0, s, V.st_d, (const int *)V.cnt_g, (const int *)V.nm_g, (const unsigned *)V.adj_g, (const int *)V.mem_g,
                           R2_ADJW, Enew, h->EP[1 - cur], h->ecap, V.mail_d + (seq % R2_MAILS), seq);
        HIP_TRY(hipGetLastError());
        cur = 1 - cur;
        *seq_out = seq; *sub_out = S_ub;
        return 0;
    };
    auto prepare = [&](bool ahead) -> int {
        const int nv = h->nv + (ahead ? gv : 0), ne = h->ne + (ahead ? ge : 0);
        const int nbv = (vm_count(h->P, std::min(nv, h->P.cap)) + PB - 1) / PB, nbe = std::max(1, (std::min(ne, h->ecap) + PB - 1) / PB);
        const size_t pool_need = (size_t)h->poolused + (size_t)(ahead ? 4 : 1) * 65536;
        if (ahead) {
            if (nbe + nbv + 2 > h->bsumcap || pool_need > h->poolcap || h->ecap > h->ecountcap) return -1;
            return 0;
        }
        if ((rc = ensure_pool(h, pool_need + (depth ? 8 * 65536 : 0)))) return rc;
        if (h->ecap > h->ecountcap) { if ((rc = grow(&h->ecount, 0, (size_t)h->ecap, s))) return rc; h->ecountcap = h->ecap; }
        const int nbv2 = (vm_count(h->P, std::min(h->nv + 2 * gv, h->P.cap)) + PB - 1) / PB, nbe2 = std::max(1, (std::min(h->ne + 2 * ge, h->ecap) + PB - 1) / PB);
        if ((rc = ensure_bsum(h, std::max(nbe + nbv, depth ? nbe2 + nbv2 : 0) + 2))) return rc;
        return 0;
    };
    for (;;) {
        while (!stop_enq && (int)inflight.size() <= depth) {
            const bool ahead = !inflight.empty();
            const int pr = prepare(ahead);
            if (pr < 0) break;
            if (pr > 0) return pr;
            int sq = 0, sub = 0;
            if ((rc = launch_round(ahead, &sq, &sub))) return rc;
            inflight.emplace_back(sq, sub);
        }
        if (inflight.empty()) break;
        int seq = inflight.front().first;
        const int S_ub = inflight.front().second;
        inflight.pop_front();
        const int nv = h->nv, ne = h->ne;
        RState m;
        if ((rc = r2_wait(h, V, seq, &m))) return rc;
        if (m.halt == 2) {
            if ((rc = drain())) return rc;
            HIP_TRY(hipMemsetAsync(V.anym, 0, (nw32 + 2) * sizeof(unsigned), s));
            HIP_TRY(hipMemsetAsync(V.bad, 0, (nw32 + 2) * sizeof(unsigned), s));
            if (mis) {
                HIP_TRY(hipMemsetAsync(V.M, 0, (size_t)Bc * nw * sizeof(unsigned), s));
                HIP_TRY(hipMemsetAsync(V.mcnt, 0, (size_t)Bc * sizeof(int), s));
            }
            if ((rc = clear_halt())) return rc;
            gv *= 4; ge *= 4;
            h->r2_spec_void++;
            continue;
        }
        if (dbg) fprintf(stderr, "r2 round %d: S %d alive %d redundant %d | go %d declined %d nminus %d nzero %d nsurv %d ncross %d pairs %d eover %d k2abort %d | nv %d ne %d pool %u\n",
                         m.round, m.S, m.nalive, m.nredundant, m.go, m.declined, m.nminus, m.nzero, m.nsurv, m.ncross, m.epairs, m.eover, m.k2abort, m.nv, m.ne, m.poolused);
        if (m.err && getenv("BSLV_R2_DEBUG")) {
            for (int which = 0; which < 2; which++) {
                const int el = m.err_info[1 + which], k = m.err_info[4];
                unsigned char fl = 0; int tcv = -7, ownv = -7; unsigned long long wm = 0, we = 0; signed char cl = 0; int co = -7;
                (void)hipMemcpy(&fl, h->P.flag + el, 1, hipMemcpyDeviceToHost);
                (void)hipMemcpy(&tcv, R.tc + el, 4, hipMemcpyDeviceToHost);
                (void)hipMemcpy(&ownv, V.own + el, 4, hipMemcpyDeviceToHost);
                (void)hipMemcpy(&co, R.cutof + el, 4, hipMemcpyDeviceToHost);
                (void)hipMemcpy(&cl, h->P.cls + el, 1, hipMemcpyDeviceToHost);
                (void)hipMemcpy(&wm, h->clsw + (size_t)(k >> 5) * h->P.cap + el, 8, hipMemcpyDeviceToHost);
                (void)hipMemcpy(&we, V.hw + (size_t)el * nw + (k >> 5), 8, hipMemcpyDeviceToHost);
                std::vector<double> hp(d + 3), x(d);
                (void)hipMemcpy(hp.data(), h->hps_d + (size_t)k * (d + 3), (d + 3) * 8, hipMemcpyDeviceToHost);
                for (int c = 0; c < d; c++) (void)hipMemcpy(&x[c], h->P.X + (size_t)c * h->P.cap + el, 8, hipMemcpyDeviceToHost);
                double sdot = 0; for (int c = 0; c < d; c++) sdot = fma(hp[c], x[c], sdot);
                int hvpos = -1;
                { std::vector<int> hv(h->P.nhv); if (h->P.nhv) (void)hipMemcpy(hv.data(), h->hv_d, (size_t)h->P.nhv * 4, hipMemcpyDeviceToHost); for (int t = 0; t < h->P.nhv; t++) if (hv[t] == el) hvpos = t; }
                fprintf(stderr, "r2 debug: element %d flag %d tc %d own %d cutof %d cls %d | class of cut %d: word-major %d, element-major %d | s %.17g alpha %.17g hi %.17g lo %.17g | position in hot list %d (nhv %d, nv_base %d, nv %d, cap %d)\n",
                        el, fl, tcv, ownv, co, cl, k, (int)((wm >> (2 * (k & 31))) & 3), (int)((we >> (2 * (k & 31))) & 3), sdot, hp[d], hp[d + 1], hp[d + 2], hvpos, h->P.nhv, h->P.nv_base, h->nv, h->P.cap);
            }
        }
        if (m.err == 4) {
            {
                const int el = m.err_info[3];
                std::vector<int> hv(std::max(h->P.nhv, 1));
                if (h->P.nhv) (void)hipMemcpy(hv.data(), h->hv_d, (size_t)h->P.nhv * 4, hipMemcpyDeviceToHost);
                int dups = 0, nondec = 0;
                std::string pos;
                for (int t = 0; t < h->P.nhv; t++) { if (hv[t] == el) pos += " " + std::to_string(t); if (t && hv[t] <= hv[t - 1]) nondec++; }
                std::vector<int> sorted(hv.begin(), hv.begin() + h->P.nhv); std::sort(sorted.begin(), sorted.end());
                for (int t = 1; t < h->P.nhv; t++) dups += sorted[t] == sorted[t - 1];
                std::vector<int> mem((size_t)std::max(m.nzero, 1));
                (void)hipMemcpy(mem.data(), h->members, (size_t)m.nzero * 4, hipMemcpyDeviceToHost);
                fprintf(stderr, "r2 debug: element %d in the hot list at:%s; hot list: %d entries, %d duplicates, %d not ascending; nv_base %d nv %d host nv %d; on-plane list:", el, pos.c_str(), h->P.nhv, dups, nondec,
                        h->P.nv_base, m.nv, h->nv);
                for (int t = 0; t < m.nzero; t++) fprintf(stderr, " %d", mem[t]);
                fprintf(stderr, "\n");
            }
            set_error("internal: round %d: member list of selected cut %d holds element %d twice (positions %d, %d); in the on-plane list at %d and %d of %d", m.round, m.err_info[0],
                      m.err_info[3], m.err_info[1], m.err_info[2], m.err_info[4], m.err_info[5], m.err_info[6]);
            return BSLV_E_STATE;
        }
        if (m.err == 3) {
            set_error("internal: round %d: the prune of selected cut %d emitted the pair (%d, %d) of its %d members: both are element %d (nzero %d)", m.err_info[6], m.err_info[0],
                      m.err_info[1], m.err_info[2], m.err_info[3], m.err_info[4], m.err_info[5]);
            return BSLV_E_STATE;
        }
        if (m.err) {
            set_error("internal: round %d: inconsistent crossing edge %d (minus end %d, plus end %d, selected cut %d = classified %d, classes %d, flag %d) hb %g hd %g a2 %g ideal %g xm %g %g %g %g xp %g %g %g %g nv_base %d nhv %d",
                      m.round, m.err_info[0], m.err_info[1], m.err_info[2], m.err_info[3], m.err_info[4], m.err_info[5], m.err_info[6],
                      m.err_d[0], m.err_d[1], m.err_d[2], m.err_d[3], m.err_d[4], m.err_d[5], m.err_d[6], m.err_d[7], m.err_d[8], m.err_d[9], m.err_d[10], m.err_d[11], h->P.nv_base, h->P.nhv);
            return BSLV_E_STATE;
        }
        if (m.stuck) { set_error("internal: a round selected no cut although %d are alive", m.nalive); return BSLV_E_STATE; }
        const bool removed_some = m.nredundant > nredundant;
        nredundant = m.nredundant;
        if (m.S == 0) {
            if ((rc = drain())) return rc;
            if ((m.halt || m.halt2) && (rc = clear_halt())) return rc;
            if (m.nalive == 0) break;
            if (removed_some) continue;
            set_error("internal: a round selected no cut although %d are alive", m.nalive);
            return BSLV_E_STATE;
        }
        if (m.declined) {
            h->r2_declined++;
            if ((rc = drain())) return rc;
            if ((rc = clear_halt())) return rc;
            hipLaunchKernelGGL(k_r2_undo, dim3((Bc + 255) / 256), dim3(256), 0, s, Bc, V.alive, (const unsigned *)V.alive_prev, (const int *)V.selmap, V.st_d);
            HIP_TRY(hipGetLastError());
            if (nv + m.ncross > h->P.cap) { stop = true; break; }
            if ((rc = ensure_pool(h, (size_t)h->poolused + (size_t)m.newlen + (size_t)m.zero_ub + 65536))) return rc;
            continue;
        }
        rounds++;
        napplied = m.napplied;
        h->ecur = 1 - h->ecur;
        h->ne = m.ne_next;
        if (m.eover || m.k2abort > 0) {
            if ((rc = drain())) return rc;
            if ((rc = clear_halt())) return rc;
        }
        if (m.eover) {
            if ((rc = ensure_ecap(h, m.ne_next + m.epairs + 1))) return rc;
            seq = ++V.seq;
            hipLaunchKernelGGL(k_r2_k2emit, dim3(S_ub), dim3(K2T), 0, s, V.st_d, (const int *)V.cnt_g, (const int *)V.nm_g, (const unsigned *)V.adj_g,
                               (const int *)V.mem_g, R2_ADJW, h->E[h->ecur], h->EP[h->ecur], h->ecap, V.mail_d + (seq % R2_MAILS), seq);
            HIP_TRY(hipGetLastError());
            if ((rc = r2_wait(h, V, seq, &m))) return rc;
            if (m.eover) { set_error("internal: the edge list is still too short after growing"); return BSLV_E_STATE; }
            if (m.k2abort > 0 && (rc = clear_halt())) return rc;
        }
        max_dv = std::max(max_dv, m.nv - nv); max_de = std::max(max_de, m.ne - ne);
        gv = std::max(gv, 2 * max_dv + 2048); ge = std::max(ge, 2 * max_de + 4096);
        h->nv = m.nv; h->ne = m.ne; h->poolused = m.poolused;
        h->new_vertices += m.ncross;
        last_ncross = m.ncross;
        if (m.k2abort > 0) {
            if ((rc = pull_order(napplied))) return rc;
            std::vector<int> cnt(m.S), nmv(m.S);
            HIP_TRY(hipMemcpy(cnt.data(), V.cnt_g, (size_t)m.S * sizeof(int), hipMemcpyDeviceToHost));
            HIP_TRY(hipMemcpy(nmv.data(), V.nm_g, (size_t)m.S * sizeof(int), hipMemcpyDeviceToHost));
            for (int sidx = 0; sidx < m.S; sidx++) if (cnt[sidx] < 0) {
                h->r2_fb_reason[std::min(4, -cnt[sidx])]++;
                int lg = 0; while ((1 << (lg + 1)) <= std::max(1, nmv[sidx]) && lg < 19) lg++;
                h->r2_fb_nm[lg]++;
            }
            const int nv0 = m.nv_next - m.ncross;
            if (m.nzero > 0) HIP_TRY(hipMemcpyAsync(R.zlist, h->members, (size_t)m.nzero * sizeof(int), hipMemcpyDeviceToDevice, s));
            for (int sidx = 0; sidx < m.S; sidx++) {
                if (cnt[sidx] >= 0) continue;
                hipLaunchKernelGGL(k_r2_gather, dim3(1), dim3(1024), 0, s, h->P, (const int *)R.zlist, m.nzero, nv0, m.ncross, (const int *)R.cutof, sidx, h->members, V.gout, m.rank_base);
                HIP_TRY(hipMemcpyAsync(V.gout_h, V.gout, 2 * sizeof(int), hipMemcpyDeviceToHost, s));
                HIP_TRY(hipStreamSynchronize(s));
                const int nm = V.gout_h[0];
                const long long len_ub = V.gout_h[1];
                if (next_counter_slot(h) < 0) { set_error("hipMemsetAsync failed"); return BSLV_E_NODEVICE; }
                h->pair_tests += (long)nm * (nm - 1) / 2;
                h->r2_fallback_prunes++;
                const int ne_before = h->ne;
                if (nm >= 2 && (rc = k2_multi(h, nm, len_ub, (int)(4 * h->cutseq + 3)))) return rc;
                if (mis && h->ne > ne_before) {
                    const int nadd = h->ne - ne_before, nbd = (nadd + PB - 1) / PB, myrank = m.rank_base + sidx;
                    if ((rc = ensure_bsum(h, nbd + 1))) return rc;
                    Tri td;
                    hipLaunchKernelGGL(k_r2_dedupe_flags, dim3(nbd), dim3(PB), 0, s, h->P, (const int *)R.cutof, (const int2 *)h->E[h->ecur], ne_before, nadd, myrank, h->bsum);
                    if ((rc = scan_totals(h, nbd, &td))) return rc;
                    if (td.a < nadd) {
                        int2 *scratch = h->E[1 - h->ecur];
                        hipLaunchKernelGGL(k_r2_dedupe_emit, dim3(nbd), dim3(PB), 0, s, h->P, (const int *)R.cutof, (const int2 *)h->E[h->ecur], ne_before, nadd, myrank, (const Tri *)h->bsum, scratch);
                        HIP_TRY(hipGetLastError());
                        if (td.a > 0) HIP_TRY(hipMemcpyAsync(h->E[h->ecur] + ne_before, scratch, (size_t)td.a * sizeof(int2), hipMemcpyDeviceToDevice, s));
                        HIP_TRY(hipStreamSynchronize(s));
                        h->ne = ne_before + td.a;
                    }
                }
            }
            HIP_TRY(hipMemcpyAsync(&V.st_d->ne, &h->ne, sizeof(int), hipMemcpyHostToDevice, s));
            HIP_TRY(hipStreamSynchronize(s));
        }
        if ((rc = check_edges(m.k2abort ? "after a round with fallback prunes" : (m.eover ? "after a round with a second emission" : "after a round"), rounds))) return rc;
        if (h->P.cap - h->nv < 4096) { stop = true; stop_enq = true; continue; }
        max_S = std::max(max_S, m.S);
        if (h->r2_defer > 0 && m.S < h->r2_defer && m.S * 5 < max_S && m.nalive > 0 && rounds >= 4) { stop = true; stop_enq = true; h->r2_deferred = true; }
        if (h->r2_min_cuts >= 0 && m.nalive >= 8 && rounds >= 16 && napplied * 4 < rounds * 5) { stop = true; stop_enq = true; }
        if (h->r2_min_cuts > 0 && m.nalive >= 8 && rounds >= 2 && napplied < h->r2_min_cuts * rounds) { stop = true; stop_enq = true; }
    }
    if (h->r2_deferred && h->r2_defer_mark) {
        const int nel = vm_count(h->P, h->nv);
        HIP_TRY(hipMemsetAsync(V.gout, 0, sizeof(int), s));
        if (nel > 0) hipLaunchKernelGGL(k_r2_mark_doomed, dim3((nel + PB - 1) / PB), dim3(PB), 0, s, h->P, (const unsigned long long *)V.hw, mis ? (const unsigned *)V.wm : (const unsigned *)nullptr, nw, h->nv,
                                        (const unsigned *)V.alive, V.gout);
        HIP_TRY(hipGetLastError());
        HIP_TRY(hipMemcpyAsync(V.gout_h, V.gout, sizeof(int), hipMemcpyDeviceToHost, s));
        HIP_TRY(hipStreamSynchronize(s));
        h->r2_doomed += V.gout_h[0];
    }
    if ((rc = pull_order(napplied))) return rc;
    std::vector<int> rcf(Bc);
    std::vector<unsigned> alive(nw32 + 2);
    HIP_TRY(hipMemcpy(rcf.data(), V.rcflag, (size_t)Bc * sizeof(int), hipMemcpyDeviceToHost));
    HIP_TRY(hipMemcpy(alive.data(), V.alive, (size_t)nw32 * sizeof(unsigned), hipMemcpyDeviceToHost));
    long long pt = 0;
    HIP_TRY(hipMemcpy(&pt, &V.st_d->pair_tests, sizeof pt, hipMemcpyDeviceToHost));
    h->pair_tests += (long)pt;
    for (int k : todo) {
        if ((alive[k >> 5] >> (k & 31)) & 1u) {
            left_out.push_back(k);
            continue;
// ... 18 lines not shown
```

### bensolve_amd/csrc/poly_rounds2_kernels.inc

```

struct RState {
    int nv, ne, nranks;
    unsigned poolused;
    int round, S, rank_base, napplied, nredundant, nalive, stuck;
    int go, declined, nminus, nzero, zero_ub, nsurv, ncross, newlen;
    int nv_next, ne_next; unsigned pool_next, pool_e, pool_z;
    int epairs, eover, k2abort;
    long long pair_tests;
    int halt;
    int halt2;
    int err, err_info[7];
    double err_d[12];
    unsigned chk;
    int seq;
};
static_assert(offsetof(RState, halt2) == offsetof(RState, halt) + sizeof(int), "k_flags2 reads (halt, halt2) as two consecutive ints");
__host__ __device__ __forceinline__ unsigned rstate_sum(const RState &s, int seq)
{
    const unsigned *w = reinterpret_cast<const unsigned *>(&s);
    unsigned c = 0x9E3779B9u;
    for (unsigned i = 0; i < sizeof(RState) / 4; i++) c = c * 31u + w[i];
    return c + (unsigned)seq * 2654435761u;
}
__device__ __forceinline__ void rstate_publish(RState *st, RState *mail, int seq)
// ... 736 lines not shown
        cand = cand && !pick && !blocked;
        const unsigned long long bc = __ballot(cand);
        if (lane == 0) { s_cand[2 * wv] = (unsigned)bc; s_cand[2 * wv + 1] = (unsigned)(bc >> 32); }
        if (!__syncthreads_or(cand ? 1 : 0)) break;
    }
    const int napplied0 = st->napplied;
    const int s = selected, r = red, keep = a && !selected && !red;
    Tri tot;
    const Tri ex = block_exscan(Tri{s, r, keep}, &tot, lds);
    if (k < Bc) {
        selmap[k] = s ? ex.a : -1;
        if (s) { sel[ex.a] = k; order[napplied0 + ex.a] = k; rcflag[k] = 0; }
        if (r) rcflag[k] = 1;
    }
    const unsigned long long ba = __ballot(a), bk = __ballot(keep), bs = __ballot(s);
    if (lane == 0) {
        const int w0 = 2 * wv;
        if (w0 < nw) { alive_prev[w0] = (unsigned)ba; alive[w0] = (unsigned)bk; selw_g[w0] = (unsigned)bs; }
        if (w0 + 1 < nw) { alive_prev[w0 + 1] = (unsigned)(ba >> 32); alive[w0 + 1] = (unsigned)(bk >> 32); selw_g[w0 + 1] = (unsigned)(bs >> 32); }
    }
    if (tid == 0) {
        st->round += 1;
        st->S = tot.a;
        st->rank_base = st->nranks;
        st->nranks += tot.a;
        st->napplied = napplied0 + tot.a;
        st->nredundant += tot.b;
        st->nalive = tot.c;
        st->stuck = (tot.a == 0 && tot.b == 0 && tot.c > 0) ? 1 : 0;
        st->go = 0; st->declined = 0; st->epairs = 0; st->eover = 0; st->k2abort = 0; st->ncross = 0; st->nzero = 0;
        if (spec && tot.a == 0) st->halt = 3;
    }
}
__global__ __launch_bounds__(PB) void k_r2_assign3(PolyView P, const unsigned long long *__restrict__ words, const unsigned *__restrict__ wm, int nw, const RState *st,
                                                   const unsigned *__restrict__ selw_g, const int *__restrict__ selmap, int *cutof, int *counters, int *zlist)
{
    __shared__ unsigned selw[32];
    if (r2_halted(st)) return;
    if (threadIdx.x < 32) selw[threadIdx.x] = (int)threadIdx.x < nw ? selw_g[threadIdx.x] : 0u;
    __syncthreads();
    const int idx = blockIdx.x * PB + threadIdx.x;
    int isminus = 0, iszero = 0, zlen = 0;
    if (idx < vm_count(P, st->nv)) {
        const int i = vm_id(P, idx);
        signed char c = 2;
        int s = -1;
        if (P.flag[i] & F_USED) {
            c = 1;
            unsigned m = st->S > 0 ? wm[i] : 0u;
            int nown = 0, ofirst = -1, ominus = -1;
            while (m) {
                const int w = __ffs((int)m) - 1;
                m &= m - 1;
                if (!selw[w]) continue;
                const unsigned long long word = words[(size_t)i * nw + w];
                const unsigned t = r2_touch32(word) & selw[w];
                if (!t) continue;
                const unsigned mn = r2_minus32(word) & selw[w];
                if (mn) ominus = w * 32 + __ffs((int)mn) - 1;
                if (ofirst < 0) ofirst = w * 32 + __ffs((int)t) - 1;
                nown += __popc(t);
            }
            if (ominus >= 0) { c = -1; s = selmap[ominus]; isminus = 1; }
            else if (nown > 0) {
                c = 0; iszero = 1;
                s = nown == 1 ? selmap[ofirst] : -1 - nown;
                zlen = zero_room(P, i, nown);
                if (nown == 1 && P.inc_len[i] > LONGN) { const int k = atomicAdd(&counters[3], 1); if (k < ZMAX) zlist[k] = i; }
            }
        }
        P.cls[i] = c;
        cutof[i] = s;
    }
    const unsigned long long bm = __ballot(isminus), bz = __ballot(iszero);
    if (bz) {
#pragma unroll
        for (int o = 32; o > 0; o >>= 1) zlen += __shfl_xor(zlen, o, WAVE);
    }
    if ((threadIdx.x & 63) == 0) {
        if (bm) atomicAdd(&counters[0], __popcll(bm));
        if (bz) { atomicAdd(&counters[1], __popcll(bz)); atomicAdd(&counters[2], zlen); }
    }
}
template <int D>
__device__ __forceinline__ void r2_classify3_body(const PolyView &P, const double *__restrict__ hps, int B, int nw, int nwp, const RState *st, const unsigned *__restrict__ alive,
                                                  unsigned long long *__restrict__ hw, unsigned *__restrict__ wm, int *mcnt, int block, int nblocks, int nthr, int packed = 1)
{
    if (!st->go || r2_halted(st)) return;
    const int vpb = nthr / nwp, w = threadIdx.x & (nwp - 1), lv = threadIdx.x / nwp, lane = threadIdx.x & 63;
    const int ncross = st->ncross, first = st->nv_next - ncross;
    const int d = D > 0 ? D : P.d;
    const unsigned aw = w < nw ? alive[w] : 0u;
    for (int base = block * vpb; base < ncross; base += nblocks * vpb) {
        const bool act = base + lv < ncross;
        const int i = first + base + lv;
        unsigned touch = 0u;
        if (act && aw) {
            double x[D > 0 ? D : MAXD];
#pragma unroll
            for (int k = 0; k < (D > 0 ? D : MAXD); k++) x[k] = k < d ? P.X[(size_t)k * P.cap + i] : 0.0;
            const bool ideal = P.flag[i] & F_IDEAL;
            const int bend = min(32, B - w * 32);
            unsigned plus = 0, notminus = 0;
            for (int bb = 0; bb < bend; bb++) {
                const double *h = hps + (size_t)(w * 32 + bb) * (d + 3);
                double s = 0.0;
#pragma unroll
                for (int k = 0; k < (D > 0 ? D : MAXD); k++) if (k < d) s = fma(h[k], x[k], s);
                const double hi = ideal ? 0.0 + POLY_EPS : h[d + 1], lo = ideal ? 0.0 - POLY_EPS : h[d + 2];
                plus |= (unsigned)(s > hi) << bb;
                notminus |= (unsigned)(s > lo) << bb;
            }
            const unsigned valid = bend == 32 ? 0xFFFFFFFFu : ((1u << bend) - 1u);
            const unsigned lowb = (plus | ~notminus) & valid, highb = notminus & valid;
            hw[(size_t)i * nw + w] = packed ? (unsigned long long)(lowb ^ highb) | ((unsigned long long)(lowb & ~highb) << 32) : spread32(lowb) | (spread32(highb) << 1);
            touch = (lowb ^ highb) & aw;
            unsigned mi = mcnt ? (lowb & ~highb & aw) : 0u;
            while (mi) { const int b = __ffs((int)mi) - 1; mi &= mi - 1; atomicAdd(&mcnt[w * 32 + b], 1); }
        }
        const unsigned long long bt = __ballot(touch != 0u);
        if (act && w == 0) wm[i] = (unsigned)((bt >> (lane & ~(nwp - 1))) & (nwp == 32 ? 0xFFFFFFFFull : ((1ull << nwp) - 1ull)));
    }
}
template <int D>
__global__ __launch_bounds__(PB) void k_r2_classify3(PolyView P, const double *__restrict__ hps, int B, int nw, int nwp, const RState *st, const unsigned *__restrict__ alive,
                                                     unsigned long long *__restrict__ hw, unsigned *__restrict__ wm, int *mcnt, int packed)
{
    r2_classify3_body<D>(P, hps, B, nw, nwp, st, alive, hw, wm, mcnt, (int)blockIdx.x, (int)gridDim.x, PB, packed);
}
template <int D>
__global__ __launch_bounds__(K2T) void k_r2_prune_classify(PolyView P, int *members, int *fcount, int *flocal, int lds_words, int2 *E, Tri *totals, Mail *mail, unsigned long long *dbg,
                                                           int *abort_flag, Hp hn, K2V2 V, const double *__restrict__ hps, int B, int nw, int nwp, const unsigned *__restrict__ alive,
                                                           unsigned long long *__restrict__ hw, unsigned *__restrict__ wm, int G, int nthr, int packed)
{
    const int S = max(V.st->S, 0), b = (int)blockIdx.x;
    if (b >= S) {
        if (b < S + G && (int)threadIdx.x < nthr) r2_classify3_body<D>(P, hps, B, nw, nwp, V.st, alive, hw, wm, (int *)nullptr, b - S, G, nthr, packed);
        if (b > 0) return;
    }
    k2_fused_body<true>(P, members, 0, 0, 0, fcount, flocal, lds_words, E, 0, (int *)nullptr, totals, mail, 0, dbg, (const CutDev *)nullptr, abort_flag, (int *)nullptr, hn, (int *)nullptr,
                        (int *)nullptr, V);
}

__global__ __launch_bounds__(PB) void k_r2_mark_doomed(PolyView P, const unsigned long long *__restrict__ hw, const unsigned *__restrict__ wm, int nw, int nv,
                                                       const unsigned *__restrict__ alive, int *count)
{
    const int idx = blockIdx.x * PB + threadIdx.x;
    if (idx >= vm_count(P, nv)) return;
    const int i = vm_id(P, idx);
    const unsigned char fl = P.flag[i];
    if (!(fl & F_USED) || (fl & F_SLTN)) return;
    unsigned m = wm ? wm[i] : 0xFFFFFFFFu;
    bool doomed = false;
    for (int w = 0; w < nw && !doomed; w++) {
        if (!((m >> w) & 1u) || alive[w] == 0u) continue;
        const unsigned long long word = hw[(size_t)i * nw + w];
        doomed = ((wm ? r2_minus32(word) : compress32(word & ~(word >> 1))) & alive[w]) != 0u;
    }
    if (doomed) { P.flag[i] = fl | F_SLTN; atomicAdd(count, 1); }
}

__global__ __launch_bounds__(PB) void k_r2_words(PolyView P, const unsigned long long *__restrict__ words, int nw, int nv, unsigned long long *__restrict__ hw)
{
    const long long t = (long long)blockIdx.x * PB + threadIdx.x;
    const int w = (int)(t % nw);
    const long long idx = t / nw;
    if (idx >= vm_count(P, nv)) return;
    const int i = vm_id(P, (int)idx);
    hw[(size_t)i * nw + w] = words[(size_t)w * P.cap + i];
}

__global__ __launch_bounds__(K2T) void k_r2_k2emit(RState *st, const int *__restrict__ cnt_g, const int *__restrict__ nm_g, const unsigned *__restrict__ adj_g,
                                                   const int *__restrict__ mem_g, int adjw_cap, int2 *E, int *EP, int ecap, RState *mail, int seq)
{
    __shared__ Tri lds[16];
    __shared__ int s_carry;
    const int S = st->S, s = blockIdx.x, tid = threadIdx.x;
    const int h2 = st->halt2;
    if (S <= 0 || !st->go || st->halt || (h2 != 0 && h2 != seq)) {
        if (s == 0 && tid == 0) rstate_publish(st, mail, seq);
        return;
    }
    Tri part{0, 0, 0};
    for (int k = tid; k < S; k += K2T) { const int c = cnt_g[k]; if (c > 0) { part.b += c; if (k < s) part.a += c; } if (c < 0) part.c += 1; }
    part = block_sum(part, lds);
    const int ebase = st->ne_next, before = part.a, total = part.b;
    const bool over = (long long)ebase + total > ecap;
    if (s == 0 && tid == 0) {
        st->epairs = total; st->eover = over; st->k2abort = part.c;
        if (over || part.c > 0) st->halt2 = seq;
        if (!over) { st->nv = st->nv_next; st->ne = ebase + total; st->poolused = st->pool_next; }
        rstate_publish(st, mail, seq);
    }
    if (over || s >= S) return;
    const int cnt = cnt_g[s];
    if (cnt <= 0) return;
    const int nm = nm_g[s];
    const int nadjw = (int)(((long long)nm * (nm - 1) / 2 + 31) / 32);
    const unsigned *adj = adj_g + (size_t)s * adjw_cap;
    const int *mem = mem_g + (size_t)s * K2_MAXNM;
    if (tid == 0) s_carry = 0;
    __syncthreads();
    for (int w0 = 0; w0 < nadjw; w0 += K2T) {
        const int ww = w0 + tid;
        unsigned word = ww < nadjw ? adj[ww] : 0u;
        Tri t{(int)__popc(word), 0, 0};
        Tri tot;
        const Tri ex = block_exscan(t, &tot, lds);
        int at = ebase + before + s_carry + ex.a;
        while (word) {
            const int bbit = __ffs((int)word) - 1;
            word &= word - 1;
            int i, j;
            pair_decode32(ww * 32 + bbit, nm, i, j);
            E[at] = int2{mem[i], mem[j]};
            if (EP) EP[at] = -1;
            at++;
        }
        __syncthreads();
        if (tid == 0) s_carry += tot.a;
        __syncthreads();
    }
}

__global__ __launch_bounds__(1024) void k_r2_gather(PolyView P, const int *zsrc, int nzero, int nv0, int ncross, const int *cutof, int s, int *members, int *out ,
                                                    int rank_base)
{
    __shared__ Tri lds[16];
    __shared__ int s_base, s_len;
    if (threadIdx.x == 0) { s_base = 0; s_len = 0; }
    __syncthreads();
    for (int c0 = 0; c0 < nzero + ncross; c0 += 1024) {
        const int c = c0 + threadIdx.x;
        int v = -1;
        if (c < nzero + ncross) { v = c < nzero ? zsrc[c] : nv0 + (c - nzero); if (!k2v2_member(P, v, cutof[v], s, rank_base + s)) v = -1; }
        Tri t{v >= 0, v >= 0 ? P.inc_len[v] : 0, 0};
        Tri tot;
        const Tri ex = block_exscan(t, &tot, lds);
        if (v >= 0) members[s_base + ex.a] = v;
        __syncthreads();
        if (threadIdx.x == 0) { s_base += tot.a; s_len += tot.b; }
        __syncthreads();
    }
    if (threadIdx.x == 0) { out[0] = s_base; out[1] = s_len; }
}

__device__ __forceinline__ bool r2_pair_is_later(const PolyView &P, const int *cutof, int2 pr, int myrank)
{
    const int cu = cutof[pr.x], cv = cutof[pr.y];
    if (cu >= -1 || cv >= -1) return false;
    const int ku = -1 - cu, kv = -1 - cv;
    const int *tu = P.pool + P.inc_off[pr.x] + P.inc_len[pr.x] - ku, *tv = P.pool + P.inc_off[pr.y] + P.inc_len[pr.y] - kv;
    for (int a = 0; a < ku; a++) { const int g = tu[a]; if (g <= myrank) continue; for (int b = 0; b < kv; b++) if (tv[b] == g) return true; }
    return false;
}
__global__ __launch_bounds__(PB) void k_r2_dedupe_flags(PolyView P, const int *cutof, const int2 *E, int e0, int n, int myrank, Tri *bsum)
{
    __shared__ Tri lds[16];
    const int k = blockIdx.x * PB + threadIdx.x;
    Tri t{0, 0, 0};
    if (k < n) t.a = r2_pair_is_later(P, cutof, E[e0 + k], myrank) ? 0 : 1;
    Tri tot;
    (void)block_exscan(t, &tot, lds);
    if (threadIdx.x == 0) bsum[blockIdx.x] = tot;
}
__global__ __launch_bounds__(PB) void k_r2_dedupe_emit(PolyView P, const int *cutof, const int2 *E, int e0, int n, int myrank, const Tri *bpre, int2 *out)
{
    __shared__ Tri lds[16];
    const int k = blockIdx.x * PB + threadIdx.x;
    Tri t{0, 0, 0};
    int2 pr{0, 0};
    if (k < n) { pr = E[e0 + k]; t.a = r2_pair_is_later(P, cutof, pr, myrank) ? 0 : 1; }
    Tri tot;
    const Tri ex = block_exscan(t, &tot, lds);
    if (t.a) out[bpre[blockIdx.x].a + ex.a] = pr;
}

__global__ void k_r2_check_edges(PolyView P, const int2 *E, int ne, int *out )
{
    const int e = blockIdx.x * blockDim.x + threadIdx.x;
    if (e >= ne) return;
    const int2 ed = E[e];
    const bool ok = (P.flag[ed.x] & F_USED) && (P.flag[ed.y] & F_USED) && ed.x != ed.y;
    if (!ok && atomicAdd(&out[0], 1) == 0) { out[1] = e; out[2] = ed.x; out[3] = ed.y; }
}
```

### bensolve_amd/poly.py

```python
import ctypes
import numpy as np
from ._lib import load_library, check

CONE_POLAR, LOWER2UPPER, UPPER2LOWER = 0, 1, 2
_bound = False


def _bind(lib):
    global _bound
    if _bound:
        return
    vp, i = ctypes.c_void_p, ctypes.c_int
    lib.bslv_poly_create.argtypes = [ctypes.POINTER(vp), i, i, vp]
    lib.bslv_poly_destroy.argtypes = [vp]
    lib.bslv_poly_destroy.restype = None
    lib.bslv_poly_dual0_apex.argtypes = [vp]
    lib.bslv_poly_add.argtypes = [vp, vp, i, vp]
    lib.bslv_poly_add_cuts.argtypes = [vp, i, vp, vp, vp]
    lib.bslv_poly_init.argtypes = [vp, vp]
    lib.bslv_poly_set_batch_mode.argtypes = [vp, i]
    lib.bslv_poly_rounds_run.argtypes = [vp]
    lib.bslv_poly_rounds_run.restype = ctypes.c_long
    lib.bslv_poly_debug_set.argtypes = [vp, ctypes.c_int, ctypes.c_long]
    lib.bslv_poly_debug_set.restype = ctypes.c_int
    lib.bslv_poly_path_stats.argtypes = [vp, vp]
    lib.bslv_poly_path_stats.restype = ctypes.c_int
    lib.bslv_poly_next.argtypes = [vp, vp, vp, vp, vp]
    lib.bslv_poly_unprocessed.argtypes = [vp, i, vp, vp, vp, vp]
    lib.bslv_poly_mark.argtypes = [vp, i, vp]
    lib.bslv_poly_dual_adjacency.argtypes = [vp]
    lib.bslv_poly_classify_batch.argtypes = [vp, i, vp, vp, vp, i, vp]
    if hasattr(lib, "bslv_poly_classify_batch_touch"):
        lib.bslv_poly_classify_batch_touch.argtypes = [vp, i, vp, vp, vp, vp]
    lib.bslv_poly_bench_fill.argtypes = [vp, i, ctypes.c_ulonglong]
    for n in ("dim", "nprimal", "ndual"):
        getattr(lib, "bslv_poly_" + n).argtypes = [vp]
    for n in ("nedges", "ninc", "ndual_edges", "pair_tests", "new_vertices"):
        f = getattr(lib, "bslv_poly_" + n)
        f.argtypes = [vp]
        f.restype = ctypes.c_long
    lib.bslv_poly_get_primal.argtypes = [vp, vp, vp, vp, vp]
    lib.bslv_poly_get_dual.argtypes = [vp, vp, vp, vp]
    lib.bslv_poly_get_edges.argtypes = [vp, vp]
    lib.bslv_poly_get_inc.argtypes = [vp, vp]
    lib.bslv_poly_get_dual_edges.argtypes = [vp, vp]
    _bound = True


class PolyEngine:

    def __init__(self, dim, v2h=CONE_POLAR, c=None):
        self.lib = load_library()
        _bind(self.lib)
        self.d = dim
        cc = None if c is None else np.ascontiguousarray(c, np.float64)
        h = ctypes.c_void_p()
        check(self.lib.bslv_poly_create(ctypes.byref(h), dim, v2h, None if cc is None else cc.ctypes.data))
        self.h = h

    def close(self):
        if getattr(self, "h", None):
            self.lib.bslv_poly_destroy(self.h)
            self.h = None

    def __del__(self):
        try:
            self.close()
        except Exception:
            pass

    def dual0_apex(self):
        check(self.lib.bslv_poly_dual0_apex(self.h))

    def add(self, val, ideal=0):
        v = np.ascontiguousarray(val, np.float64)
        rc = ctypes.c_int()
        check(self.lib.bslv_poly_add(self.h, v.ctypes.data, int(ideal), ctypes.byref(rc)))
        return rc.value

    def add_cuts(self, vals, ideals=None):
        vals = np.ascontiguousarray(vals, np.float64).reshape(-1, self.d)
        B = len(vals)
        rc = np.zeros(B, np.int32)
        idl = None if ideals is None else np.ascontiguousarray(ideals, np.int32)
        check(self.lib.bslv_poly_add_cuts(self.h, B, vals.ctypes.data, None if idl is None else idl.ctypes.data, rc.ctypes.data))
        return rc

    def set_batch_mode(self, mode):
        check(self.lib.bslv_poly_set_batch_mode(self.h, int(mode)))

    def rounds_run(self):
        return self.lib.bslv_poly_rounds_run(self.h)

    def debug_set(self, key, value):
        check(self.lib.bslv_poly_debug_set(self.h, int(key), int(value)))

    def rounds2_stats(self):
        out = (ctypes.c_long * 5)()
        self.lib.bslv_poly_rounds2_stats.argtypes = [ctypes.c_void_p, ctypes.c_void_p]
        check(self.lib.bslv_poly_rounds2_stats(self.h, out))
        return dict(rounds=out[0], cuts=out[1], chunks=out[2], fallback_prunes=out[3], declined=out[4])

    def rounds2_health(self):
        for f in ("bslv_poly_rounds2_late_left", "bslv_poly_rounds2_torn_reads"):
            getattr(self.lib, f).restype = ctypes.c_long
            getattr(self.lib, f).argtypes = [ctypes.c_void_p]
        return dict(late_left=self.lib.bslv_poly_rounds2_late_left(self.h), torn_reads=self.lib.bslv_poly_rounds2_torn_reads(self.h))

    def sharded_prunes(self):
        self.lib.bslv_poly_sharded_prunes.restype = ctypes.c_long
        self.lib.bslv_poly_sharded_prunes.argtypes = [ctypes.c_void_p]
        return self.lib.bslv_poly_sharded_prunes(self.h)

    def set_prune_window(self, blocks):
        self.lib.bslv_poly_set_prune_window.argtypes = [ctypes.c_void_p, ctypes.c_long]
        check(self.lib.bslv_poly_set_prune_window(self.h, int(blocks)))

    def get_prune_window(self):
        self.lib.bslv_poly_get_prune_window.restype = ctypes.c_long
        self.lib.bslv_poly_get_prune_window.argtypes = [ctypes.c_void_p]
        return self.lib.bslv_poly_get_prune_window(self.h)

    def prune_window_stats(self):
        out = (ctypes.c_long * 3)()
        self.lib.bslv_poly_prune_window_stats.argtypes = [ctypes.c_void_p, ctypes.c_void_p]
        check(self.lib.bslv_poly_prune_window_stats(self.h, out))
        return list(out)

    @staticmethod
    def selftest_pair_blocks(nm, window_blocks=0, samples=100000):
        lib = load_library()
        out = (ctypes.c_long * 4)()
        lib.bslv_selftest_pair_blocks.argtypes = [ctypes.c_int, ctypes.c_long, ctypes.c_int, ctypes.c_void_p]
        check(lib.bslv_selftest_pair_blocks(int(nm), int(window_blocks), int(samples), out))
        return list(out)

    def set_snap(self, on=1):
        self.lib.bslv_poly_set_snap.argtypes = [ctypes.c_void_p, ctypes.c_int]
        check(self.lib.bslv_poly_set_snap(self.h, on))

    def snapped(self):
        out = ctypes.c_long()
        self.lib.bslv_poly_snapped.argtypes = [ctypes.c_void_p, ctypes.c_void_p]
        check(self.lib.bslv_poly_snapped(self.h, ctypes.byref(out)))
        return out.value

    def path_stats(self):
        out = (ctypes.c_long * 6)()
        check(self.lib.bslv_poly_path_stats(self.h, out))
        return dict(hot_chunks=out[0], speculative=out[1], declined=out[2], prune_fallbacks=out[3], single_cuts=out[4], member_list_prunes=out[5])

    def init(self):
        rc = ctypes.c_int()
        check(self.lib.bslv_poly_init(self.h, ctypes.byref(rc)))
        return rc.value

    def next(self):
        v = np.empty(self.d)
        ideal, idx, rc = ctypes.c_int(), ctypes.c_int(), ctypes.c_int()
        check(self.lib.bslv_poly_next(self.h, v.ctypes.data, ctypes.byref(ideal), ctypes.byref(idx), ctypes.byref(rc)))
        return None if rc.value else (v, ideal.value, idx.value)

    def unprocessed(self, max_out=None):
        cnt = ctypes.c_int()
        check(self.lib.bslv_poly_unprocessed(self.h, 0, None, None, None, ctypes.byref(cnt)))
        n = cnt.value if max_out is None else min(cnt.value, max_out)
        idx = np.empty(n, np.int32)
        val = np.empty((n, self.d))
        ideal = np.empty(n, np.int32)
        if n:
            check(self.lib.bslv_poly_unprocessed(self.h, n, idx.ctypes.data, val.ctypes.data, ideal.ctypes.data, ctypes.byref(cnt)))
        return idx, val, ideal, cnt.value

    def mark(self, idx):
        idx = np.ascontiguousarray(np.atleast_1d(idx), np.int32)
        check(self.lib.bslv_poly_mark(self.h, len(idx), idx.ctypes.data))

    def dual_adjacency(self):
        check(self.lib.bslv_poly_dual_adjacency(self.h))

    def classify_batch(self, hps, repeats=1, fetch=True):
        hps = np.ascontiguousarray(hps, np.float64).reshape(-1, self.d + 1)
        B = len(hps)
        nv = self.lib.bslv_poly_nprimal(self.h)
        words = np.zeros(((B + 31) // 32, nv), np.uint64) if fetch else None
# ... 96 lines not shown
```

### include/bslv_hip.h

```cpp
#ifndef BSLV_HIP_H
#define BSLV_HIP_H

#include <stddef.h>
#include <stdint.h>

#ifdef __cplusplus
extern "C" {
#endif

enum {
    BSLV_OK = 0,
    BSLV_E_NODEVICE = 1,
    BSLV_E_ARG = 2,
    BSLV_E_NOMEM = 3,
    BSLV_E_CAPACITY = 4,
    BSLV_E_STATE = 5
};

enum { BSLV_LP_INFEASIBLE = 0, BSLV_LP_UNBOUNDED = 1, BSLV_LP_UNEXPECTED = 2, BSLV_LP_UNDEFINED = 3, BSLV_LP_OPTIMAL = 4 };

const char *bslv_last_error(void);
int bslv_device_count(void);
int bslv_set_device(int device);
int bslv_device_info(char *name, int name_len, int *cus, size_t *mem_bytes);
// ... 44 lines not shown
int  bslv_lpq_solve_batch_method(bslv_lpq *h, int method, int B, const int *src, const int *dst,
                                 const double *vlo, const double *vup, int *status, int *iters);
int  bslv_lpq_solve_batch_obj(bslv_lpq *h, int B, const int *src, const int *dst, const double *vlo, const double *vup,
                              int cost_first, int cost_cnt, const double *costs, int *status, int *iters);
int  bslv_lpq_get_primal(bslv_lpq *h, int B, const int *slot, int first, int cnt, double *out);
int  bslv_lpq_get_dual(bslv_lpq *h, int B, const int *slot, int first, int cnt, double *out);
int  bslv_lpq_get_obj(bslv_lpq *h, int B, const int *slot, double *out);
int bslv_lpq_certify(bslv_lpq *h, int B, const int *slot,
                     const double *vlo, const double *vup,
                     int cost_first, int cost_cnt, const double *costs,
                     const double *tol,
                     double *res,
                     int *at,
                     int *verdict);
int bslv_lpq_last_certify_stats(const bslv_lpq *h, long out[3]);
int bslv_lpq_debug_poke(bslv_lpq *h, int slot, int what, int var, double delta);
enum { BSLV_LP_RAY_NONE = 0, BSLV_LP_RAY_FARKAS = 1, BSLV_LP_RAY_DIRECTION = 2 };
int bslv_lpq_set_rays(bslv_lpq *h, int on);
int bslv_lpq_get_rays(const bslv_lpq *h);
int bslv_lpq_get_ray(bslv_lpq *h, int B, const int *slot, int *kind , double *ray );
int bslv_lpq_last_ray_stats(const bslv_lpq *h, long out[3]);
int bslv_lpq_certify_rays(bslv_lpq *h, int B, const int *slot, const double *vlo, const double *vup,
                          int cost_first, int cost_cnt, const double *costs, const double *tol ,
                          double *res , int *at , int *verdict );
int bslv_lpq_last_ray_certify_stats(const bslv_lpq *h, long out[3]);
int  bslv_lpq_set_profile(bslv_lpq *h, int on);
int  bslv_lpq_last_stats(const bslv_lpq *h, int *lockstep_iters, long *pivots, double *update_ms, double *total_ms);
long bslv_lpq_last_passes(const bslv_lpq *h);
long bslv_lpq_last_launches(const bslv_lpq *h);
int  bslv_lpq_last_ext_stats(const bslv_lpq *h, long out[4]);
long bslv_lpq_last_flip_updates(const bslv_lpq *h);
long bslv_lpq_last_init_chunks(const bslv_lpq *h);
int  bslv_lpq_set_extended(bslv_lpq *h, int on);
int  bslv_lpq_get_extended(const bslv_lpq *h);
enum { BSLV_LP_METHOD_DUAL = 0, BSLV_LP_METHOD_PRIMAL = 1, BSLV_LP_METHOD_REPAIR = 2 };
int  bslv_lpq_set_method(bslv_lpq *h, int method);
int  bslv_lpq_get_method(const bslv_lpq *h);
int  bslv_lpq_last_phase1_stats(const bslv_lpq *h, long out[3]);
enum { BSLV_LP_PRICING_DANTZIG = 0, BSLV_LP_PRICING_DEVEX = 1 };
int  bslv_lpq_set_pricing(bslv_lpq *h, int rule);
int  bslv_lpq_get_pricing(const bslv_lpq *h);
int  bslv_lpq_last_pricing_stats(const bslv_lpq *h, long out[3]);
int  bslv_lpq_last_pricing_norms(bslv_lpq *h, int b, double *s);
int  bslv_lpq_set_primal_pricing(bslv_lpq *h, int rule);
int  bslv_lpq_get_primal_pricing(const bslv_lpq *h);
int  bslv_lpq_last_primal_pricing_stats(const bslv_lpq *h, long out[3]);
int  bslv_lpq_last_primal_pricing_norms(bslv_lpq *h, int b, double *t );
int  bslv_lpq_set_canonical(bslv_lpq *h, int on, const double *dir );
int  bslv_lpq_get_canonical(const bslv_lpq *h);
int  bslv_lpq_last_canonical_stats(const bslv_lpq *h, long out[4]);
int  bslv_lpq_solve_batch_canonical(bslv_lpq *h, const double *dir , int B, const int *src, const int *dst,
                                    const double *vlo, const double *vup, int *status, int *iters);
int  bslv_lpq_set_canonical_obj(bslv_lpq *h, int on, int cost_first, int cost_cnt, const double *ddir );
int  bslv_lpq_get_canonical_obj(const bslv_lpq *h);
int  bslv_lpq_last_canonical_obj_stats(const bslv_lpq *h, long out[4]);
int  bslv_lpq_solve_batch_obj_canonical(bslv_lpq *h, const double *ddir , int B, const int *src, const int *dst,
                                        const double *vlo, const double *vup, int cost_first, int cost_cnt, const double *costs,
                                        int *status, int *iters);

typedef struct bslv_poly bslv_poly;

int  bslv_poly_create(bslv_poly **out, int dim, int v2h, const double *c );
void bslv_poly_destroy(bslv_poly *h);
int  bslv_poly_dual0_apex(bslv_poly *h);
int  bslv_poly_add(bslv_poly *h, const double *val, int ideal, int *rc_out);
int  bslv_poly_add_cuts(bslv_poly *h, int B, const double *val , const int *ideal ,
                        int *rc_out );
int  bslv_poly_set_batch_mode(bslv_poly *h, int mode);
long bslv_poly_rounds_run(const bslv_poly *h);
int  bslv_poly_path_stats(const bslv_poly *h, long out[6]);
long bslv_poly_sharded_prunes(const bslv_poly *h);
int  bslv_poly_set_snap(bslv_poly *h, int on);
int  bslv_poly_snapped(bslv_poly *h, long *moved);
int  bslv_poly_largest_facet(const bslv_poly *h);
long bslv_poly_noflag_prunes(const bslv_poly *h);
int  bslv_poly_set_prune_window(bslv_poly *h, long blocks);
long bslv_poly_get_prune_window(const bslv_poly *h);
int  bslv_poly_prune_window_stats(const bslv_poly *h, long out[3]);
long bslv_poly_rounds2_late_left(const bslv_poly *h);
long bslv_poly_rounds2_torn_reads(const bslv_poly *h);
int  bslv_poly_set_defer(bslv_poly *h, int min_cuts);
int  bslv_poly_debug_set(bslv_poly *h, int key, long value);
int  bslv_poly_rounds2_stats(const bslv_poly *h, long out[5]);
int  bslv_poly_init(bslv_poly *h, int *rc_out);
int  bslv_poly_next(bslv_poly *h, double *val, int *ideal, int *idx, int *rc_out);
int  bslv_poly_unprocessed(bslv_poly *h, int max_out, int *idx, double *val, int *ideal, int *count);
int  bslv_poly_unprocessed2(bslv_poly *h, int max_out, int from_end, int *idx, double *val, int *ideal, int *parent, int *count);
int  bslv_poly_children_hist(bslv_poly *h, int first_facet, int n, int *counts, int *total, int *older);
int  bslv_poly_children_of(bslv_poly *h, int nfacets, const int *facets, int max_out, int *idx, double *val, int *ideal, int *parent, int *n_out);
int  bslv_poly_mark(bslv_poly *h, int n, const int *idx);
int  bslv_poly_dual_adjacency(bslv_poly *h);
int  bslv_poly_classify_batch(bslv_poly *h, int B, const double *hps, unsigned long long *words_out,
                              int *anyminus_out, int repeats, float *ms_out);
int  bslv_poly_classify_batch_touch(bslv_poly *h, int B, const double *hps, unsigned long long *words_out, int *tc_out, int *t1_out);
int  bslv_poly_bench_fill(bslv_poly *h, int nv, unsigned long long seed);
int  bslv_poly_dim(const bslv_poly *h);
int  bslv_poly_nprimal(const bslv_poly *h);
int  bslv_poly_ndual(const bslv_poly *h);
long bslv_poly_nedges(const bslv_poly *h);
long bslv_poly_ninc(bslv_poly *h);
long bslv_poly_ndual_edges(const bslv_poly *h);
long bslv_poly_pair_tests(const bslv_poly *h);
long bslv_poly_new_vertices(const bslv_poly *h);
int  bslv_poly_get_primal(bslv_poly *h, unsigned char *used, unsigned char *ideal, unsigned char *sltn, double *coords);
int  bslv_poly_get_dual(bslv_poly *h, unsigned char *used, unsigned char *ideal, double *coords);
int  bslv_poly_get_primal_range(bslv_poly *h, int first, int count, double *coords);
int  bslv_poly_get_edges(bslv_poly *h, int *ab);
int  bslv_poly_get_inc(bslv_poly *h, int *pairs);
int  bslv_poly_get_dual_edges(bslv_poly *h, int *ab);
int  bslv_poly_check(bslv_poly *h, double tol , int row_first, int row_count ,
                     long out[12], double worst[2] ,
                     int *offenders , int max_off, int *n_off);
int  bslv_poly_debug_corrupt(bslv_poly *h, int what, int a, int b, double x);
int  bslv_poly_garbage(bslv_poly *h, long out[6]);
int  bslv_poly_compact(bslv_poly *h, int *new_of_old , long out[6] );
int  bslv_poly_last_compact_stats(const bslv_poly *h, long out[8]);
int  bslv_selftest_mailbox(int which, int rounds, long *torn_out);
int  bslv_selftest_pair_blocks(int nm, long window_blocks, int samples, long out[4]);

typedef struct bslv_benson bslv_benson;

int  bslv_benson_create(bslv_benson **out, int m, int n, int q, const double *A, const double *P,
                        const char *rtype, const double *rlb, const double *rub,
                        const char *ctype, const double *clb, const double *cub,
                        const double *R, int r, const double *c, double eps, int pool_slots);
int  bslv_benson_create_ex(bslv_benson **out, int m, int n, int q, const double *A, const double *P,
                           const char *rtype, const double *rlb, const double *rub,
                           const char *ctype, const double *clb, const double *cub,
                           const double *R, int r, const double *c, const double *eta, int hom, int flags, double eps, int pool_slots);
enum { BSLV_BENSON_PREIMAGES = 2 };
int  bslv_benson_preimage_p(const bslv_benson *h, int element, double *x );
int  bslv_benson_preimage_d(const bslv_benson *h, int facet, double *uw );
int  bslv_benson_set_preimage_p(bslv_benson *h, int element, const double *x );
void bslv_benson_destroy(bslv_benson *h);
int  bslv_benson_start(bslv_benson *h, int *vlp_status );
int  bslv_benson_collect(bslv_benson *h, int max_batch, int rank, int world, int *n_local, int *n_total);
int  bslv_benson_record_len(const bslv_benson *h);
int  bslv_benson_solve_local(bslv_benson *h, double *records, int *pivots_out, int *lockstep_out);
int  bslv_benson_apply(bslv_benson *h, int nrec, const double *records, long *stats );
int  bslv_benson_step(bslv_benson *h, int max_batch, long *stats , double *ms );
int  bslv_benson_set_pipelined(bslv_benson *h, int on);
int  bslv_benson_collect_ctx(bslv_benson *h, int ctx, int max_batch, int rank, int world, int *n_local, int *n_total);
int  bslv_benson_solve_local_ctx(bslv_benson *h, int ctx, double *records, int *pivots_out, int *lockstep_out);
int  bslv_benson_apply_ctx(bslv_benson *h, int ctx, int nrec, const double *records, long *stats);
int  bslv_benson_unprocessed_left(const bslv_benson *h);
int  bslv_benson_set_canonical(bslv_benson *h, int on);
int  bslv_benson_get_canonical(const bslv_benson *h);
int  bslv_benson_canonical_stats(const bslv_benson *h, long last[4], long total[4]);
int  bslv_benson_set_certify(bslv_benson *h, int on);
int  bslv_benson_get_certify(const bslv_benson *h);
int  bslv_benson_certify_stats(const bslv_benson *h, long counts[3], double worst[5]);
int  bslv_benson_set_compact(bslv_benson *h, double dead_fraction , long min_slots );
int  bslv_benson_compact_stats(const bslv_benson *h, long out[4]);
int  bslv_benson_set_policy(bslv_benson *h, int policy);
int  bslv_benson_set_sibling_rule(bslv_benson *h, int cap, int window);
int  bslv_benson_set_fronts(bslv_benson *h, int nfronts, int sib_cap);
int  bslv_benson_set_families(bslv_benson *h, int mode, int batches);
int  bslv_benson_set_defer(bslv_benson *h, int min_cuts);
int  bslv_benson_defer_stats(const bslv_benson *h, long out[4]);
int  bslv_benson_collect_given(bslv_benson *h, int n, const int *idx, const double *val, const int *parent, int rank, int world, int *n_local, int *n_total);
int  bslv_benson_last_local(bslv_benson *h, int max_out, int *src, int *pivots, int *gen);
int  bslv_benson_pool_stats(bslv_benson *h, long out[4]);
int  bslv_benson_resident_slots(bslv_benson *h, int max_out, int *slots, int *gen);
int  bslv_benson_set_park(bslv_benson *h, int on);
int  bslv_benson_park_stats(const bslv_benson *h, long out[5]);
int  bslv_benson_totals(const bslv_benson *h, long *lps, long *cuts, long *pivots);
// ... 62 lines not shown
```

Measured before the change: 163,900.

## Split large prune pair sweeps across helper workgroups and stage hyperplanes in LDS

Adds helper workgroups to the rounds2 prune/classify kernel. Each helper builds a histogram of member counts per prune, assigns itself to one of the largest prunes, and sweeps a strided subset of the pair rows there, merging adjacency bits with atomicOr and reporting partial counts. The emit kernel then sums those counts and clears the adjacency words. Separately, the classify path can stage the hyperplane batch into LDS with a padded transposed layout. Both aim to cut tail latency from a few large prunes, at the cost of redundant membership scans, extra atomics and more blocks per launch.

Result: faster. 167,300, median of 6 (+2.1%).

```diff
diff --git a/bensolve_amd/csrc/poly_engine.hip b/bensolve_amd/csrc/poly_engine.hip
--- a/bensolve_amd/csrc/poly_engine.hip
+++ b/bensolve_amd/csrc/poly_engine.hip
@@ -1493,7 +1493,7 @@
 }
 template <int NWC>
 __device__ __forceinline__ void k2_pairs(int nm, int d, int W, int NW, const unsigned long long *bits, const unsigned long long *rows, unsigned *adj_bits,
-                                         int (*queue)[128], const unsigned long long *later = nullptr)
+                                         int (*queue)[128], const unsigned long long *later = nullptr, int part = 0, int nparts = 1)
 {
     const int lane = threadIdx.x & 63, wave = threadIdx.x >> 6;
     auto sweep = [&](int p) {
@@ -1518,7 +1518,7 @@
     };
     int qn = 0;
     int *q = queue[wave];
-    for (int i = wave; i < nm - 1; i += K2T / WAVE) {
+    for (int i = part * (K2T / WAVE) + wave; i < nm - 1; i += nparts * (K2T / WAVE)) {
         const int rowbase = i * (2 * nm - i - 1) / 2 - (i + 1);
         for (int j0 = i + 1; j0 < nm; j0 += WAVE) {
             const int j = j0 + lane;
@@ -1548,7 +1548,10 @@
 struct K2V2 {
     const RState *st; const int *cutof; int *mem_g; unsigned *adj_g; int *cnt_g; int *nm_g; int adjw_cap; long long *pair_tests;
     int *fc2, *fl2, *fc_ticket; int fc_slices, fc_stride;
+    int *npart_g, *cntx_g; int helpers, split_min, split_parts;
+    int *split_stat;
 };
+constexpr int K2_MAXPARTS = 4, K2_SPLIT_MAXS = 1024, K2_DBG_SLOTS = 32, K2_DBG_LARGE = 192;
 __device__ __forceinline__ int k2v2_round(const RState *st);
 __device__ __forceinline__ int k2v2_rank_base(const RState *st);
 __device__ __forceinline__ bool k2v2_member(const PolyView &P, int v, int co, int vs, int want)
@@ -1560,20 +1563,45 @@
     for (int t = 0; t < k; t++) mine |= tail[t] == want;
     return mine;
 }
+__device__ __forceinline__ void k2v2_count_owners(const PolyView &P, int v, int co, int rank_base, int S, int *hist)
+{
+    if (co >= -1) { if (co >= 0 && co < S) atomicAdd(&hist[co], 1); return; }
+    const int k = -1 - co;
+    const int *tail = P.pool + P.inc_off[v] + P.inc_len[v] - k;
+    for (int t = 0; t < k; t++) { const int s = tail[t] - rank_base; if (s >= 0 && s < S) atomicAdd(&hist[s], 1); }
+}
+__device__ __forceinline__ int k2v2_parts(const K2V2 &V, int n)
+{
+    return n >= V.split_min && n <= K2_MAXNM ? min(min(V.split_parts, K2_MAXPARTS), 1 + n / max(V.split_min, 2)) : 1;
+}
+__device__ __forceinline__ void k2v2_assign(const K2V2 &V, const int *nm, int S, int vs, int helper, int *out)
+{
+    for (int s = threadIdx.x; s < S; s += K2T) {
+        const int n = nm[s], want = k2v2_parts(V, n) - 1;
+        if (want <= 0 || (helper < 0 && s != vs)) continue;
+        int off = 0;
+        for (int k = 0; k < S; k++) { const int nk = nm[k]; if (nk > n || (nk == n && k < s)) off += k2v2_parts(V, nk) - 1; }
+        const int got = max(0, min(want, V.helpers - off));
+        if (helper < 0) out[2] = 1 + got;
+        else if (helper >= off && helper < off + got) { out[0] = s; out[1] = 1 + helper - off; out[2] = 1 + got; }
+    }
+}
 __device__ __forceinline__ void k2v2_sizes(const RState *st, int &S, int &go, int &nzero, int &nv0, int &ncross);
 __device__ void k2v2_check_members(const K2V2 &V, int vs, const int *s_mem, int nm, const int *members, int nzero);
 template <bool V2>
 __device__ void k2_fused_body(PolyView P, int *members, int nzero, int nv0, int ncross, int *fcount, int *flocal,
                               int lds_words, int2 *E, int ebase, int *ne_dev, Tri *totals, Mail *mail, int seq, unsigned long long *dbg,
-                              const CutDev *cd, int *abort_flag, int *EP, const Hp &hn, int *counters_n, int *zlist_n, const K2V2 &V)
+                              const CutDev *cd, int *abort_flag, int *EP, const Hp &hn, int *counters_n, int *zlist_n, const K2V2 &V, int helper = -1)
 {
     extern __shared__ unsigned long long k2_dyn[];
+    int S = 0;
     if (V2) {
-        int S, go;
+        int go;
         k2v2_sizes(V.st, S, go, nzero, nv0, ncross);
         if (blockIdx.x == 0 && threadIdx.x == 0 && V.fc_ticket) V.fc_ticket[(k2v2_round(V.st) + 1) & 1] = 0;
-        if (!go || (int)blockIdx.x >= S) return;
+        if (!go || S <= 0 || (helper < 0 && (int)blockIdx.x >= S)) return;
         cd = nullptr; ne_dev = nullptr;
+        if (helper >= 0) dbg = nullptr;
     }
     if (!V2 && blockIdx.x > 0) {
         classify_body(P, hn, cd->nv_new, counters_n, zlist_n, (blockIdx.x - 1) * K2T + threadIdx.x);
@@ -1596,6 +1624,7 @@
         }
     }
     unsigned long long t_prev = dbg ? wall_clock64() : 0ull;
+    const unsigned long long t_start = t_prev;
 #define K2_PHASE(k) do { if (dbg && threadIdx.x == 0) { unsigned long long t_now = wall_clock64(); if (V2) atomicAdd(&dbg[k], t_now - t_prev); else dbg[k] += t_now - t_prev; t_prev = t_now; } } while (0)
     __shared__ Tri lds[16];
     __shared__ unsigned s_off[K2_MAXNM];
@@ -1605,15 +1634,41 @@
     __shared__ int s_queue[K2T / WAVE][128];
     const int tid = threadIdx.x, d = P.d;
     int nm = nzero + ncross;
-    const int vs = (int)blockIdx.x;
-    const int myrank = V2 ? k2v2_rank_base(V.st) + vs : 0x7FFFFFFF;
-    auto v2_result = [&](int cnt, int n) { if (tid == 0) { V.cnt_g[vs] = cnt; V.nm_g[vs] = n; } };
+    int vs = (int)blockIdx.x;
+    int part = 0, nparts = 1;
+    int myrank = V2 ? k2v2_rank_base(V.st) + vs : 0x7FFFFFFF;
+    auto v2_result = [&](int cnt, int n) {
+        if (tid != 0) return;
+        if (part == 0) { V.cnt_g[vs] = cnt; V.nm_g[vs] = n; V.npart_g[vs] = nparts; }
+        else if (cnt >= 0) V.cntx_g[vs * (K2_MAXPARTS - 1) + part - 1] = cnt;
+    };
     if (V2) {
-        __shared__ int s_base;
-        if (tid == 0) s_base = 0;
+        __shared__ int s_base, s_asg[3];
+        __shared__ int s_hist[K2_SPLIT_MAXS];
+        const bool split = V.helpers > 0 && V.split_parts > 1 && S <= K2_SPLIT_MAXS;
+        if (helper >= 0 && !split) return;
+        if (split) for (int k = tid; k < S; k += K2T) s_hist[k] = 0;
+        if (tid == 0) { s_base = 0; s_asg[0] = -1; s_asg[1] = 0; s_asg[2] = 1; }
         __syncthreads();
-        const int ncand = nzero + ncross;
+        const int ncand = nzero + ncross, rank_base = k2v2_rank_base(V.st);
         constexpr int CPT = 8;
+        const bool one_trip = ncand <= K2T * CPT;
+        auto learn = [&]() {
+            __syncthreads();
+            k2v2_assign(V, s_hist, S, vs, helper, s_asg);
+            __syncthreads();
+            nparts = s_asg[2];
+            if (helper < 0) return true;
+            vs = s_asg[0]; part = s_asg[1]; myrank = rank_base + vs;
+            return vs >= 0;
+        };
+        if (helper >= 0 && !one_trip)
+            for (int c0 = 0; c0 < ncand; c0 += K2T * CPT)
+#pragma unroll
+                for (int u = 0; u < CPT; u++) {
+                    const int c = c0 + tid * CPT + u;
+                    if (c < ncand) { const int v = c < nzero ? members[c] : nv0 + (c - nzero); k2v2_count_owners(P, v, V.cutof[v], rank_base, S, s_hist); }
+                }
         for (int c0 = 0; c0 < ncand; c0 += K2T * CPT) {
             const int cb = c0 + tid * CPT;
             int vv[CPT], co[CPT], cnt = 0;
@@ -1621,6 +1676,11 @@
             for (int u = 0; u < CPT; u++) { const int c = cb + u; vv[u] = c < ncand ? (c < nzero ? members[c] : nv0 + (c - nzero)) : -1; }
 #pragma unroll
             for (int u = 0; u < CPT; u++) co[u] = vv[u] >= 0 ? V.cutof[vv[u]] : 0;
+            if (split && (helper < 0 || one_trip)) {
+#pragma unroll
+                for (int u = 0; u < CPT; u++) if (vv[u] >= 0) k2v2_count_owners(P, vv[u], co[u], rank_base, S, s_hist);
+            }
+            if (helper >= 0 && c0 == 0 && !learn()) return;
 #pragma unroll
             for (int u = 0; u < CPT; u++) { if (vv[u] >= 0 && !k2v2_member(P, vv[u], co[u], vs, myrank)) vv[u] = -1; cnt += vv[u] >= 0; }
             Tri t{cnt, 0, 0};
@@ -1633,13 +1693,15 @@
             if (tid == 0) s_base += tot.a;
             __syncthreads();
         }
+        if (helper >= 0 && ncand == 0) return;
+        if (helper < 0 && split) learn();
         nm = s_base;
         K2_PHASE(10);
         if (nm > K2_MAXNM) { v2_result(-1, nm); return; }
 #ifdef BSLV_R2_CHECK_MEMBERS
         k2v2_check_members(V, vs, s_mem, nm, members, nzero);
 #endif
-        if (tid == 0 && nm >= 2) atomicAdd((unsigned long long *)V.pair_tests, (unsigned long long)((long long)nm * (nm - 1) / 2));
+        if (tid == 0 && part == 0 && nm >= 2) atomicAdd((unsigned long long *)V.pair_tests, (unsigned long long)((long long)nm * (nm - 1) / 2));
         if (nm < 2) { v2_result(0, nm); return; }
     }
     const long long npairs = (long long)nm * (nm - 1) / 2;
@@ -1678,6 +1740,10 @@
     }
     __syncthreads();
     const bool use_hash = 2 * s_total <= K2_HASH && (long long)K2_HASH <= bits_cap;
+    if (V2 && !use_hash && nparts > 1) {
+        if (part > 0) return;
+        nparts = 1;
+    }
     if (V2 && !use_hash) {
         __shared__ int s_slice;
         if (tid == 0) s_slice = V.fc_slices > 0 ? atomicAdd(&V.fc_ticket[k2v2_round(V.st) & 1], 1) : V.fc_slices;
@@ -1749,23 +1815,32 @@
     if (!use_hash) k2_for_entries(P.pool, nm, s_off, s_len, s_islong, s_long, nlong, [&](int, int g) { fcount[g] = 0; });
     K2_PHASE(3);
     const unsigned long long *lat = V2 ? later : nullptr;
-    if (NW <= 1) k2_pairs<1>(nm, d, W, NW, bits, rows, adj_bits, s_queue, lat);
-    else if (NW <= 2) k2_pairs<2>(nm, d, W, NW, bits, rows, adj_bits, s_queue, lat);
-    else if (NW <= 4) k2_pairs<4>(nm, d, W, NW, bits, rows, adj_bits, s_queue, lat);
-    else k2_pairs<K2_MAXNM / 64>(nm, d, W, NW, bits, rows, adj_bits, s_queue, lat);
+    const unsigned long long t_p4 = t_prev;
+    if (NW <= 1) k2_pairs<1>(nm, d, W, NW, bits, rows, adj_bits, s_queue, lat, part, nparts);
+    else if (NW <= 2) k2_pairs<2>(nm, d, W, NW, bits, rows, adj_bits, s_queue, lat, part, nparts);
+    else if (NW <= 4) k2_pairs<4>(nm, d, W, NW, bits, rows, adj_bits, s_queue, lat, part, nparts);
+    else k2_pairs<K2_MAXNM / 64>(nm, d, W, NW, bits, rows, adj_bits, s_queue, lat, part, nparts);
     __syncthreads();
     K2_PHASE(4);
+    const unsigned long long p4_ticks = t_prev - t_p4;
     K2_PHASE(5);
     if (V2) {
         unsigned *ag = V.adj_g + (size_t)vs * V.adjw_cap;
         int *mg = V.mem_g + (size_t)vs * K2_MAXNM;
-        int part = 0;
-        for (int w = tid; w < nadjw; w += K2T) { const unsigned x = adj_bits[w]; ag[w] = x; part += __popc(x); }
-        for (int m = tid; m < nm; m += K2T) mg[m] = s_mem[m];
-        const Tri tt = block_sum(Tri{part, 0, 0}, lds);
+        int npairs_mine = 0;
+        if (nparts == 1) for (int w = tid; w < nadjw; w += K2T) { const unsigned x = adj_bits[w]; ag[w] = x; npairs_mine += __popc(x); }
+        else for (int w = tid; w < nadjw; w += K2T) { const unsigned x = adj_bits[w]; if (x) atomicOr(&ag[w], x); npairs_mine += __popc(x); }
+        if (part == 0) for (int m = tid; m < nm; m += K2T) mg[m] = s_mem[m];
+        const Tri tt = block_sum(Tri{npairs_mine, 0, 0}, lds);
         v2_result(tt.a, nm);
+        if (tid == 0 && nparts > 1) atomicAdd(&V.split_stat[part == 0 ? 0 : 1], 1);
         K2_PHASE(6);
-        if (dbg && tid == 0) { atomicAdd(&dbg[7], 1ull); atomicAdd(&dbg[8], (unsigned long long)W); atomicAdd(&dbg[9], (unsigned long long)s_nloc); atomicAdd(&dbg[11], (unsigned long long)nm); atomicMax(&dbg[12], (unsigned long long)nm); }
+        if (dbg && tid == 0) {
+            atomicAdd(&dbg[7], 1ull); atomicAdd(&dbg[8], (unsigned long long)W); atomicAdd(&dbg[9], (unsigned long long)s_nloc); atomicAdd(&dbg[11], (unsigned long long)nm); atomicMax(&dbg[12], (unsigned long long)nm);
+            const unsigned long long whole = t_prev - t_start;
+            atomicMax(&dbg[13], p4_ticks); atomicMax(&dbg[17], whole);
+            if (nm >= K2_DBG_LARGE) { atomicAdd(&dbg[14], 1ull); atomicAdd(&dbg[15], p4_ticks); atomicAdd(&dbg[16], whole); atomicAdd(&dbg[18], (unsigned long long)nm); }
+        }
         return;
     }
     int last_tot = 0;
@@ -2073,6 +2148,11 @@
     bool r2_mis = true;
     bool r2_ride = true;
     int r2_ride_gmax = 240;
+    bool r2_ride_lds = true;
+    bool r2_split = true;
+    int r2_split_min = 64;
+    int r2_split_parts = 4;
+    int r2_split_helpers = 32;
     int r2_ride_threads = 256;
     int chunk_cuts = 1024;
     int r2_defer = 0;
@@ -3011,13 +3091,18 @@
     if (const char *e = getenv("BSLV_R2_RIDE")) h->r2_ride = atoi(e) != 0;
     if (const char *e = getenv("BSLV_R2_RIDE_G")) h->r2_ride_gmax = std::max(1, atoi(e));
     if (const char *e = getenv("BSLV_R2_RIDE_T")) bslv_poly_debug_set(h, 20, atol(e));
+    if (const char *e = getenv("BSLV_R2_RIDE_LDS")) bslv_poly_debug_set(h, 22, atol(e));
+    if (const char *e = getenv("BSLV_R2_SPLIT")) bslv_poly_debug_set(h, 23, atol(e));
+    if (const char *e = getenv("BSLV_R2_SPLIT_MIN")) bslv_poly_debug_set(h, 24, atol(e));
+    if (const char *e = getenv("BSLV_R2_SPLIT_PARTS")) bslv_poly_debug_set(h, 25, atol(e));
+    if (const char *e = getenv("BSLV_R2_SPLIT_H")) bslv_poly_debug_set(h, 26, atol(e));
     if (const char *e = getenv("BSLV_CHUNK_CUTS")) h->chunk_cuts = std::min(4096, std::max(32, atoi(e)));
     if (const char *e = getenv("BSLV_R2_MIN_CUTS")) h->r2_min_cuts = std::max(-1, atoi(e));
     if (const char *e = getenv("BSLV_POLY_SNAP")) h->snap = atoi(e) != 0;
     if (const char *e = getenv("BSLV_CROSS_UB")) h->cross_ub = std::max(0, atoi(e));
     if (const char *e = getenv("BSLV_K2_LDS")) h->k2_lds = (size_t)std::max(64, atoi(e));
     if (const char *e = getenv("BSLV_K2_WINDOW")) { const long long v = atoll(e); if (v > 0) h->window_blocks = std::min(v, PAIR_WINDOW_DEFAULT); }
-    if (getenv("BSLV_K2_DEBUG") && malloc0(&h->k2dbg, 16 * sizeof(unsigned long long)) == hipSuccess) (void)hipMemset(h->k2dbg, 0, 16 * sizeof(unsigned long long));
+    if (getenv("BSLV_K2_DEBUG") && malloc0(&h->k2dbg, K2_DBG_SLOTS * sizeof(unsigned long long)) == hipSuccess) (void)hipMemset(h->k2dbg, 0, K2_DBG_SLOTS * sizeof(unsigned long long));
     h->rounds = new RoundsBuf();
     std::vector<double> z(dim, 0.0);
     z[dim - 1] = -1.0;
@@ -3044,8 +3129,12 @@
                 h->tm_launch[2] / std::max(1L, h->n_single), h->tm_launch[3] / std::max(1L, h->n_single));
     if (h->cutlog) fclose(h->cutlog);
     if (h->k2dbg) {
-        unsigned long long t[16];
-        if (hipMemcpy(t, h->k2dbg, sizeof(t), hipMemcpyDeviceToHost) == hipSuccess && t[7])
+        unsigned long long t[K2_DBG_SLOTS] = {0};
+        if (hipMemcpy(t, h->k2dbg, sizeof(t), hipMemcpyDeviceToHost) != hipSuccess) t[7] = 0;
+        if (t[7] && t[17])
+            fprintf(stderr, "k2_fused, rounds: prunes of >= %d members: %llu of %llu, members mean %.0f, P4 mean %.2f us, whole prune mean %.2f us | over all prunes: P4 max %.2f us, whole prune max %.2f us\n", K2_DBG_LARGE, t[14], t[7],
+                    t[14] ? (double)t[18] / t[14] : 0.0, t[14] ? t[15] * 0.01 / t[14] : 0.0, t[14] ? t[16] * 0.01 / t[14] : 0.0, t[13] * 0.01, t[17] * 0.01);
+        if (t[7])
             fprintf(stderr, "k2_fused phases (us/launch over %llu launches; rounds: per prune workgroup): P0a %.2f P0 %.2f P1 %.2f P2 %.2f P3 %.2f P4 %.2f P5 %.2f P6 %.2f | W %.1f nloc %.0f | members mean %.0f max %llu\n", t[7],
                     t[10] * 0.01 / t[7], t[0] * 0.01 / t[7], t[1] * 0.01 / t[7], t[2] * 0.01 / t[7], t[3] * 0.01 / t[7], t[4] * 0.01 / t[7], t[5] * 0.01 / t[7], t[6] * 0.01 / t[7], (double)t[8] / t[7], (double)t[9] / t[7],
                     (double)t[11] / t[7], t[12]);
@@ -3474,6 +3563,11 @@
     case 18: h->r2_ride = value != 0; return 0;
     case 19: h->r2_ride_gmax = (int)std::max(1L, std::min(4096L, value)); return 0;
     case 20: { int t = 64; while (t < K2T && t < value) t <<= 1; h->r2_ride_threads = t; return 0; }
+    case 22: h->r2_ride_lds = value != 0; return 0;
+    case 23: h->r2_split = value != 0; return 0;
+    case 24: h->r2_split_min = (int)std::max(2L, std::min((long)K2_MAXNM + 1, value)); return 0;
+    case 25: h->r2_split_parts = (int)std::max(2L, std::min((long)K2_MAXPARTS, value)); return 0;
+    case 26: h->r2_split_helpers = (int)std::max(1L, std::min(256L, value)); return 0;
     case 16: h->k2_noflags = value != 0; return 0;
     case 11: h->r2_mis = value != 0; return 0;
     case 14: h->r2_defer = (int)std::max(0L, value); return 0;
@@ -3633,6 +3727,11 @@
     if (!h || !out) return BSLV_E_ARG;
     out[0] = h->r2_rounds; out[1] = h->r2_cuts; out[2] = h->r2_chunks; out[3] = h->r2_fallback_prunes; out[4] = h->r2_declined;
     return 0;
+}
+int bslv_poly_split_stats(bslv_poly *h, long out[2])
+{
+    if (!h || !out) return BSLV_E_ARG;
+    return rounds2_split_stats(h, out);
 }
 int bslv_poly_bench_fill(bslv_poly *h, int nv, unsigned long long seed)
 {
diff --git a/bensolve_amd/csrc/poly_rounds2_host.inc b/bensolve_amd/csrc/poly_rounds2_host.inc
--- a/bensolve_amd/csrc/poly_rounds2_host.inc
+++ b/bensolve_amd/csrc/poly_rounds2_host.inc
@@ -10,6 +10,7 @@
     int *own = nullptr; int vcap = 0;
     unsigned long long *hw = nullptr; size_t hwcap = 0;
     int *cnt_g = nullptr, *nm_g = nullptr, *mem_g = nullptr; unsigned *adj_g = nullptr; int scap = 0;
+    int *npart_g = nullptr, *cntx_g = nullptr, *split_stat = nullptr;
     int *gout = nullptr, *gout_h = nullptr;
     int seq = 0;
     unsigned chunk_seed = 0;
@@ -24,12 +25,22 @@
 {
     auto fr = [](void *p) { if (p) (void)hipFree(p); };
     fr(V.st_d); fr(V.alive); fr(V.alive_prev); fr(V.anym); fr(V.bad); fr(V.selmap); fr(V.sel); fr(V.order); fr(V.rcflag); fr(V.own);
-    fr(V.cnt_g); fr(V.nm_g); fr(V.mem_g); fr(V.adj_g); fr(V.gout); fr(V.hw); fr(V.M); fr(V.selw); fr(V.wm); fr(V.mcnt); fr(V.fc2); fr(V.fl2); fr(V.fc_ticket);
+    fr(V.cnt_g); fr(V.nm_g); fr(V.npart_g); fr(V.cntx_g); fr(V.split_stat); fr(V.mem_g); fr(V.adj_g); fr(V.gout); fr(V.hw); fr(V.M); fr(V.selw); fr(V.wm); fr(V.mcnt); fr(V.fc2); fr(V.fl2); fr(V.fc_ticket);
     if (V.mail_h) (void)hipHostFree(V.mail_h);
     if (V.gout_h) (void)hipHostFree(V.gout_h);
     V = Rounds2Buf();
 }
 static hipError_t r2_prune_classify_grant(int d, int lds);
+static int rounds2_split_stats(bslv_poly *h, long out[2])
+{
+    int c[2] = {0, 0};
+    if (h->rounds2 && h->rounds2->split_stat) {
+        HIP_TRY(hipStreamSynchronize(h->stream));
+        HIP_TRY(hipMemcpy(c, h->rounds2->split_stat, sizeof c, hipMemcpyDeviceToHost));
+    }
+    out[0] = c[0]; out[1] = c[1];
+    return 0;
+}
 static int rounds2_ensure(bslv_poly *h, Rounds2Buf &V, int Bc)
 {
     hipStream_t s = h->stream;
@@ -40,6 +51,8 @@
         HIP_TRY(hipHostGetDevicePointer((void **)&V.mail_d, V.mail_h, 0));
         memset(V.mail_h, 0, R2_MAILS * sizeof(RState));
         HIP_TRY(malloc0(&V.gout, 4 * sizeof(int)));
+        HIP_TRY(malloc0(&V.split_stat, 2 * sizeof(int)));
+        HIP_TRY(hipMemsetAsync(V.split_stat, 0, 2 * sizeof(int), s));
         HIP_TRY(hipHostMalloc(&V.gout_h, 4 * sizeof(int)));
         HIP_TRY(malloc0(&V.M, (size_t)R2_MAXC * (R2_MAXC / 32) * sizeof(unsigned)));
         HIP_TRY(malloc0(&V.selw, 64 * sizeof(unsigned)));
@@ -65,7 +78,9 @@
         if ((rc = grow(&V.cnt_g, 0, (size_t)nc, s))) return rc;
         if ((rc = grow(&V.nm_g, 0, (size_t)nc, s))) return rc;
         if ((rc = grow(&V.mem_g, 0, (size_t)nc * K2_MAXNM, s))) return rc;
-        if ((rc = grow(&V.adj_g, 0, (size_t)nc * R2_ADJW, s))) return rc;
+        if ((rc = grow(&V.adj_g, 0, (size_t)nc * R2_ADJW, s, true))) return rc;
+        if ((rc = grow(&V.npart_g, 0, (size_t)nc, s, true))) return rc;
+        if ((rc = grow(&V.cntx_g, 0, (size_t)nc * (K2_MAXPARTS - 1), s, true))) return rc;
         V.bcap = nc; V.scap = nc;
     }
     if (h->P.cap > V.vcap) { if ((rc = grow(&V.own, 0, (size_t)h->P.cap, s))) return rc; V.vcap = h->P.cap; }
@@ -351,14 +366,17 @@
                        (const int *)h->EP[cur], h->EP[1 - cur], Z, (const unsigned long long *)V.hw, (const unsigned *)V.wm, nw, (int *)nullptr,
                        (const unsigned *)V.selw, (const int *)V.selmap);
         const int S_ub = std::max(1, std::min(Bc - napplied - nredundant, V.scap));
-        const K2V2 KV{V.st_d, R.cutof, V.mem_g, V.adj_g, V.cnt_g, V.nm_g, R2_ADJW, &V.st_d->pair_tests, V.fc2, V.fl2, V.fc_ticket, V.fc2 ? V.fc_slices : 0, V.fc_stride};
+        const K2V2 KV{V.st_d, R.cutof, V.mem_g, V.adj_g, V.cnt_g, V.nm_g, R2_ADJW, &V.st_d->pair_tests, V.fc2, V.fl2, V.fc_ticket, V.fc2 ? V.fc_slices : 0, V.fc_stride,
+                      V.npart_g, V.cntx_g, 0, h->r2_split_min, h->r2_split_parts, V.split_stat};
         const int seq = ++V.seq;
         const int want = std::max(2048, 2 * last_ncross);
         if (h->r2_ride && h->k2_lds <= V.ride_lds) {
             const int nthr = std::max(h->r2_ride_threads, std::min(nwp, K2T));
             const int vpb = std::max(1, nthr / nwp), G = std::max(1, std::min(h->r2_ride_gmax, (want + vpb - 1) / vpb));
-            launch_r2_prune_classify(d, dim3(S_ub + G), h->k2_lds, s, h->P, h->members, h->fcount, h->flocal, (int)(h->k2_lds / 8), Enew, h->totals + 2, h->k2mail_d, h->k2dbg, h->abort_d,
-                                     Hp{}, KV, (const double *)h->hps_d, Bc, nw, nwp, (const unsigned *)V.alive, V.hw, V.wm, G, nthr, mis ? 1 : 0);
+            K2V2 KH = KV;
+            KH.helpers = h->r2_split ? h->r2_split_helpers : 0;
+            launch_r2_prune_classify(d, dim3(S_ub + KH.helpers + G), h->k2_lds, s, h->P, h->members, h->fcount, h->flocal, (int)(h->k2_lds / 8), Enew, h->totals + 2, h->k2mail_d, h->k2dbg, h->abort_d,
+                                     Hp{}, KH, (const double *)h->hps_d, Bc, nw, nwp, (const unsigned *)V.alive, V.hw, V.wm, G, nthr, mis ? 1 : 0, h->r2_ride_lds ? 1 : 0);
         } else {
             launch_r2_classify3(d, dim3(std::max(1, std::min(4096, (want + PB / nwp - 1) / (PB / nwp)))), s, h->P, (const double *)h->hps_d, Bc, nw, nwp, (const RState *)V.st_d,
                                 (const unsigned *)V.alive, V.hw, V.wm, (int *)nullptr, mis ? 1 : 0);
@@ -366,8 +384,8 @@
                                (int *)nullptr, h->totals + 2, h->k2mail_d, 0, h->k2dbg, (const CutDev *)nullptr, h->abort_d, (int *)nullptr, Hp{}, (int *)nullptr,
                                (int *)nullptr, KV);
         }
-        hipLaunchKernelGGL(k_r2_k2emit, dim3(S_ub), dim3(K2T), 0, s, V.st_d, (const int *)V.cnt_g, (const int *)V.nm_g, (const unsigned *)V.adj_g, (const int *)V.mem_g,
-                           R2_ADJW, Enew, h->EP[1 - cur], h->ecap, V.mail_d + (seq % R2_MAILS), seq);
+        hipLaunchKernelGGL(k_r2_k2emit, dim3(S_ub), dim3(K2T), 0, s, V.st_d, (const int *)V.cnt_g, (const int *)V.nm_g, V.adj_g, (const int *)V.npart_g, (const int *)V.cntx_g,
+                           (const int *)V.mem_g, R2_ADJW, Enew, h->EP[1 - cur], h->ecap, V.mail_d + (seq % R2_MAILS), seq);
         HIP_TRY(hipGetLastError());
         cur = 1 - cur;
         *seq_out = seq; *sub_out = S_ub;
@@ -504,7 +522,7 @@
         if (m.eover) {
             if ((rc = ensure_ecap(h, m.ne_next + m.epairs + 1))) return rc;
             seq = ++V.seq;
-            hipLaunchKernelGGL(k_r2_k2emit, dim3(S_ub), dim3(K2T), 0, s, V.st_d, (const int *)V.cnt_g, (const int *)V.nm_g, (const unsigned *)V.adj_g,
+            hipLaunchKernelGGL(k_r2_k2emit, dim3(S_ub), dim3(K2T), 0, s, V.st_d, (const int *)V.cnt_g, (const int *)V.nm_g, V.adj_g, (const int *)V.npart_g, (const int *)V.cntx_g,
                                (const int *)V.mem_g, R2_ADJW, h->E[h->ecur], h->EP[h->ecur], h->ecap, V.mail_d + (seq % R2_MAILS), seq);
             HIP_TRY(hipGetLastError());
             if ((rc = r2_wait(h, V, seq, &m))) return rc;
diff --git a/bensolve_amd/csrc/poly_rounds2_kernels.inc b/bensolve_amd/csrc/poly_rounds2_kernels.inc
--- a/bensolve_amd/csrc/poly_rounds2_kernels.inc
+++ b/bensolve_amd/csrc/poly_rounds2_kernels.inc
@@ -842,11 +842,21 @@
         if (bz) { atomicAdd(&counters[1], __popcll(bz)); atomicAdd(&counters[2], zlen); }
     }
 }
-template <int D>
+__device__ __forceinline__ int r2_hps_lds_stride(int nw) { return nw | 1; }
+__device__ __forceinline__ void r2_stage_hps(const double *__restrict__ hps, int B, int nw, int d, double *lh)
+{
+    const int nwl = r2_hps_lds_stride(nw), n = B * (d + 3);
+    for (int e = threadIdx.x; e < n; e += blockDim.x) {
+        const int c = e / (d + 3), k = e - c * (d + 3);
+        lh[((c & 31) * (d + 3) + k) * nwl + (c >> 5)] = hps[e];
+    }
+}
+template <int D, bool LDSH = false>
 __device__ __forceinline__ void r2_classify3_body(const PolyView &P, const double *__restrict__ hps, int B, int nw, int nwp, const RState *st, const unsigned *__restrict__ alive,
                                                   unsigned long long *__restrict__ hw, unsigned *__restrict__ wm, int *mcnt, int block, int nblocks, int nthr, int packed = 1)
 {
     if (!st->go || r2_halted(st)) return;
+    const int hstride = LDSH ? r2_hps_lds_stride(nw) : 1;
     const int vpb = nthr / nwp, w = threadIdx.x & (nwp - 1), lv = threadIdx.x / nwp, lane = threadIdx.x & 63;
     const int ncross = st->ncross, first = st->nv_next - ncross;
     const int d = D > 0 ? D : P.d;
@@ -863,11 +873,11 @@
             const int bend = min(32, B - w * 32);
             unsigned plus = 0, notminus = 0;
             for (int bb = 0; bb < bend; bb++) {
-                const double *h = hps + (size_t)(w * 32 + bb) * (d + 3);
+                const double *h = LDSH ? hps + (size_t)bb * (d + 3) * hstride + w : hps + (size_t)(w * 32 + bb) * (d + 3);
                 double s = 0.0;
 #pragma unroll
-                for (int k = 0; k < (D > 0 ? D : MAXD); k++) if (k < d) s = fma(h[k], x[k], s);
-                const double hi = ideal ? 0.0 + POLY_EPS : h[d + 1], lo = ideal ? 0.0 - POLY_EPS : h[d + 2];
+                for (int k = 0; k < (D > 0 ? D : MAXD); k++) if (k < d) s = fma(h[k * hstride], x[k], s);
+                const double hi = ideal ? 0.0 + POLY_EPS : h[(d + 1) * hstride], lo = ideal ? 0.0 - POLY_EPS : h[(d + 2) * hstride];
                 plus |= (unsigned)(s > hi) << bb;
                 notminus |= (unsigned)(s > lo) << bb;
             }
@@ -891,15 +901,27 @@
 template <int D>
 __global__ __launch_bounds__(K2T) void k_r2_prune_classify(PolyView P, int *members, int *fcount, int *flocal, int lds_words, int2 *E, Tri *totals, Mail *mail, unsigned long long *dbg,
                                                            int *abort_flag, Hp hn, K2V2 V, const double *__restrict__ hps, int B, int nw, int nwp, const unsigned *__restrict__ alive,
-                                                           unsigned long long *__restrict__ hw, unsigned *__restrict__ wm, int G, int nthr, int packed)
-{
-    const int S = max(V.st->S, 0), b = (int)blockIdx.x;
-    if (b >= S) {
-        if (b < S + G && (int)threadIdx.x < nthr) r2_classify3_body<D>(P, hps, B, nw, nwp, V.st, alive, hw, wm, (int *)nullptr, b - S, G, nthr, packed);
+                                                           unsigned long long *__restrict__ hw, unsigned *__restrict__ wm, int G, int nthr, int packed, int hps_lds)
+{
+    extern __shared__ unsigned long long k2_dyn[];
+    const int S = max(V.st->S, 0), H = V.helpers, b = (int)blockIdx.x;
+    if (b >= S + H) {
+        if (b < S + H + G) {
+            const int d = D > 0 ? D : P.d;
+            const bool staged = hps_lds && (long long)r2_hps_lds_stride(nw) * 32 * (d + 3) <= (long long)lds_words && V.st->go && !r2_halted(V.st);
+            if (staged) {
+                r2_stage_hps(hps, B, nw, d, (double *)k2_dyn);
+                __syncthreads();
+            }
+            if ((int)threadIdx.x < nthr) {
+                if (staged) r2_classify3_body<D, true>(P, (const double *)k2_dyn, B, nw, nwp, V.st, alive, hw, wm, (int *)nullptr, b - S - H, G, nthr, packed);
+                else r2_classify3_body<D>(P, hps, B, nw, nwp, V.st, alive, hw, wm, (int *)nullptr, b - S - H, G, nthr, packed);
+            }
+        }
         if (b > 0) return;
     }
     k2_fused_body<true>(P, members, 0, 0, 0, fcount, flocal, lds_words, E, 0, (int *)nullptr, totals, mail, 0, dbg, (const CutDev *)nullptr, abort_flag, (int *)nullptr, hn, (int *)nullptr,
-                        (int *)nullptr, V);
+                        (int *)nullptr, V, b >= S && b > 0 ? b - S : -1);
 }
 
 __global__ __launch_bounds__(PB) void k_r2_mark_doomed(PolyView P, const unsigned long long *__restrict__ hw, const unsigned *__restrict__ wm, int nw, int nv,
@@ -930,8 +952,8 @@
     hw[(size_t)i * nw + w] = words[(size_t)w * P.cap + i];
 }
 
-__global__ __launch_bounds__(K2T) void k_r2_k2emit(RState *st, const int *__restrict__ cnt_g, const int *__restrict__ nm_g, const unsigned *__restrict__ adj_g,
-                                                   const int *__restrict__ mem_g, int adjw_cap, int2 *E, int *EP, int ecap, RState *mail, int seq)
+__global__ __launch_bounds__(K2T) void k_r2_k2emit(RState *st, const int *__restrict__ cnt_g, const int *__restrict__ nm_g, unsigned *__restrict__ adj_g,
+                                                   const int *__restrict__ npart_g, const int *__restrict__ cntx_g, const int *__restrict__ mem_g, int adjw_cap, int2 *E, int *EP, int ecap, RState *mail, int seq)
 {
     __shared__ Tri lds[16];
     __shared__ int s_carry;
@@ -942,7 +964,8 @@
         return;
     }
     Tri part{0, 0, 0};
-    for (int k = tid; k < S; k += K2T) { const int c = cnt_g[k]; if (c > 0) { part.b += c; if (k < s) part.a += c; } if (c < 0) part.c += 1; }
+    auto pairs_of = [&](int k) { int c = cnt_g[k]; if (c >= 0) for (int p = 1; p < npart_g[k]; p++) c += cntx_g[k * (K2_MAXPARTS - 1) + p - 1]; return c; };
+    for (int k = tid; k < S; k += K2T) { const int c = pairs_of(k); if (c > 0) { part.b += c; if (k < s) part.a += c; } if (c < 0) part.c += 1; }
     part = block_sum(part, lds);
     const int ebase = st->ne_next, before = part.a, total = part.b;
     const bool over = (long long)ebase + total > ecap;
@@ -953,17 +976,18 @@
         rstate_publish(st, mail, seq);
     }
     if (over || s >= S) return;
-    const int cnt = cnt_g[s];
+    const int cnt = pairs_of(s);
     if (cnt <= 0) return;
     const int nm = nm_g[s];
     const int nadjw = (int)(((long long)nm * (nm - 1) / 2 + 31) / 32);
-    const unsigned *adj = adj_g + (size_t)s * adjw_cap;
+    unsigned *adj = adj_g + (size_t)s * adjw_cap;
     const int *mem = mem_g + (size_t)s * K2_MAXNM;
     if (tid == 0) s_carry = 0;
     __syncthreads();
     for (int w0 = 0; w0 < nadjw; w0 += K2T) {
         const int ww = w0 + tid;
         unsigned word = ww < nadjw ? adj[ww] : 0u;
+        if (word) adj[ww] = 0u;
         Tri t{(int)__popc(word), 0, 0};
         Tri tot;
         const Tri ex = block_exscan(t, &tot, lds);
diff --git a/bensolve_amd/poly.py b/bensolve_amd/poly.py
--- a/bensolve_amd/poly.py
+++ b/bensolve_amd/poly.py
@@ -101,6 +101,12 @@
         check(self.lib.bslv_poly_rounds2_stats(self.h, out))
         return dict(rounds=out[0], cuts=out[1], chunks=out[2], fallback_prunes=out[3], declined=out[4])
 
+    def split_stats(self):
+        out = (ctypes.c_long * 2)()
+        self.lib.bslv_poly_split_stats.argtypes = [ctypes.c_void_p, ctypes.c_void_p]
+        check(self.lib.bslv_poly_split_stats(self.h, out))
+        return dict(split_prunes=out[0], helper_parts=out[1])
+
     def rounds2_health(self):
         for f in ("bslv_poly_rounds2_late_left", "bslv_poly_rounds2_torn_reads"):
             getattr(self.lib, f).restype = ctypes.c_long
diff --git a/include/bslv_hip.h b/include/bslv_hip.h
--- a/include/bslv_hip.h
+++ b/include/bslv_hip.h
@@ -150,6 +150,7 @@
 int  bslv_poly_set_defer(bslv_poly *h, int min_cuts);
 int  bslv_poly_debug_set(bslv_poly *h, int key, long value);
 int  bslv_poly_rounds2_stats(const bslv_poly *h, long out[5]);
+int  bslv_poly_split_stats(bslv_poly *h, long out[2]);
 int  bslv_poly_init(bslv_poly *h, int *rc_out);
 int  bslv_poly_next(bslv_poly *h, double *val, int *ideal, int *idx, int *rc_out);
 int  bslv_poly_unprocessed(bslv_poly *h, int max_out, int *idx, double *val, int *ideal, int *count);
```
